# dlavado/scene-net

Hardware: AMD Instinct MI355X
Metric: voxel-tiles/sec (point cloud -> 64^3 occupancy -> 16-GENEO bank conv -> head) (higher is better)
Workload: dtype i8; 1 GPU; C2: 32 tiles/GPU x 100000 points (fp64 xyz, UTM-scale), 64^3 voxel grid, 16 GENEO kernels 9^3 (cy 6, cone 5, neg 5); conv on the int8 matrix cores: binary occupancy x 24-bit fixed-point weights (3 int8 digits), exact int32 accumulation, fp32 head; tiles_per_gpu=32, points_per_tile=100000, geneo_kernels=16, parallelism=tile-sharded x1, no collectives

## Files before the change

### include/scenenet_hip.h

```cpp
#ifndef SCENENET_HIP_H
#define SCENENET_HIP_H

#include <stddef.h>
#include <stdint.h>

#ifdef __cplusplus
extern "C" {
#endif

typedef void* sn_stream_t;

typedef enum {
    SN_OK = 0,
    SN_ERR_INVALID_ARG = -1,
    SN_ERR_UNSUPPORTED = -2,
    SN_ERR_LAUNCH = -3,
    SN_ERR_NO_DEVICE = -4,
    SN_ERR_DEVICE_STATUS = -5
} sn_status;

typedef enum { SN_F32 = 0, SN_F64 = 1, SN_U8 = 2, SN_OCC8 = 3, SN_BF16 = 4, SN_I32 = 5 } sn_dtype;

typedef enum {
    SN_GENEO_CY = 0, SN_GENEO_CONE = 1, SN_GENEO_NEG = 2,
    SN_GENEO_CY_V1 = 3, SN_GENEO_CONE_V1 = 4, SN_GENEO_NEG_V1 = 5
} sn_geneo_kind;

enum {
    SN_P_RADIUS = 0,
    SN_P_SIGMA = 1,
    SN_P_APEX = 2,
    SN_P_CONE_RADIUS = 3,
    SN_P_CONE_INC = 4,
    SN_P_NEG_FACTOR = 5,
    SN_NPARAM = 8
};

int sn_version(void);
int sn_prepare_device(void);
int sn_device_status(int* code, int* detail2);
int sn_device_status_clear(void);
int sn_conv_i8_path_counts(unsigned long long* counts3);
const char* sn_last_error(void);

int sn_device_count(void);

int sn_set_option(const char* name, int value);
int sn_get_option(const char* name);

int sn_geneo_bank(const float* params, const int32_t* kinds, int G, int kz, int kx, int ky,
                  float* bank, int32_t* status, sn_stream_t stream);

int sn_effective_lambdas(float* lambdas, const int32_t* order, int G, int last, float* out, sn_stream_t stream);
int sn_geneo_bank_lambdas(const float* params, const int32_t* kinds, int G, int kz, int kx, int ky, float* bank,
                          int32_t* status, float* lambdas, const int32_t* order, int last, float* lambdas_out,
                          sn_stream_t stream);
int sn_geneo_bank_prep(const float* params, const int32_t* kinds, int G, int kz, int kx, int ky, float* bank,
                       int32_t* status, float* lambdas, const int32_t* order, int last, float* lambdas_out,
                       void* prep, sn_stream_t stream);

int sn_conv_bank(const void* x, int x_dtype, const float* bank, const float* lambdas,
                 int B, int Z, int X, int Y, int G, int kz, int kx, int ky,
                 void* act, void* out, int out_dtype, sn_stream_t stream);

int sn_conv_bank_plan(int x_dtype, int B, int Z, int X, int Y, int G, int kz, int kx, int ky, int32_t* plan8);

#define SN_CONV_PREP_BYTES 16384
int sn_conv_bank_prep(const float* bank, int G, int kz, int kx, int ky, void* prep, sn_stream_t stream);
int sn_conv_bank_prepared(const void* x, int x_dtype, const float* bank, const float* lambdas, void* prep,
                          int B, int Z, int X, int Y, int G, int kz, int kx, int ky,
                          void* act, void* out, int out_dtype, sn_stream_t stream);
int sn_conv_bank_prepared_served(const void* x, int x_dtype, const float* bank, const float* lambdas, void* prep,
                                 int B, int Z, int X, int Y, int G, int kz, int kx, int ky,
                                 void* act, void* out, int out_dtype, sn_stream_t stream);
int sn_conv_prep_verdict_offset(void);
int sn_conv_i8_spin_timeouts(unsigned long long* count);
int sn_conv_i8z_round_counts(unsigned long long* counts2);
int sn_voxel_onepass_giveups(unsigned long long* count);

int sn_launch_timing_events(void* start_event, void* stop_event);

int sn_conv_fused(const void* x, int x_dtype, const float* bank, const float* lambdas, int B, int Z, int X, int Y,
                  int G, int kz, int kx, int ky, void* out, int out_dtype, sn_stream_t stream);
int sn_conv_fused_v(const void* x, int x_dtype, const float* bank, const float* lambdas, int B, int Z, int X, int Y, int G,
                    int kz, int kx, int ky, void* out, int out_dtype, int32_t* verdict, int assume_served,
                    sn_stream_t stream);
size_t sn_conv_fused_prep_bytes(int kz, int kx, int ky);
int sn_conv_fused_prep(const float* bank, const float* lambdas, int G, int kz, int kx, int ky, void* blob,
                       sn_stream_t stream);
int sn_conv_fused_prepared(const void* x, int x_dtype, const float* bank, const float* lambdas, const void* blob, int B,
                           int Z, int X, int Y, int G, int kz, int kx, int ky, void* out, int out_dtype, int assume_served,
                           sn_stream_t stream);


int sn_conv_fused_supported(int B, int Z, int X, int Y, int kz, int kx, int ky);

int sn_forward_auto(const void* x, int x_dtype, const float* bank, const float* lambdas, int B, int Z, int X, int Y,
                    int G, int kz, int kx, int ky, uint8_t* occ_ws, int32_t* not_binary, void* out, int out_dtype,
                    sn_stream_t stream);


#define SN_DESC_LEN(nx, ny, nz) (6 + (nx) + (ny) + (nz) + 3)

int sn_voxel_bbox(const double* pts, const int64_t* offsets, int B, double* bbox, sn_stream_t stream);

#define SN_BBOX_PARTS 32
int sn_voxel_prepare(const double* pts, const int64_t* offsets, int B, int nx, int ny, int nz, int regular,
                     double* partial_ws, double* bbox, double* desc, sn_stream_t stream);

int sn_voxel_desc(const double* bbox, int B, int nx, int ny, int nz, int regular,
                  double* desc, sn_stream_t stream);

int sn_voxel_desc_from_bounds(const double* bounds, int B, int nx, int ny, int nz,
                              double* desc, sn_stream_t stream);

int sn_voxel_desc_sized(const double* bbox, int B, const double* size_xyz_host, int nx, int ny, int nz,
                        double* desc, int32_t* dims, int32_t* status, sn_stream_t stream);

int sn_voxel_finalize_sized(const int32_t* counts, const int32_t* tower_counts, int B, int nx, int ny, int nz,
                            const double* desc, int32_t* colstats, double* density, double* gt, float* occ,
                            float* gt_occ, sn_stream_t stream);

int sn_voxel_scatter(const double* pts, const double* labels, const int64_t* offsets, int B,
                     const double* desc, int nx, int ny, int nz,
                     int32_t* counts, int32_t* tower_counts,
                     const double* keep_labels_host, int n_keep,
                     int32_t* dropped, sn_stream_t stream);

int sn_voxel_finalize(const int32_t* counts, const int32_t* tower_counts, int B, int nx, int ny, int nz,
                      int32_t* colstats, double* density, double* gt, float* occ, float* gt_occ,
                      sn_stream_t stream);

#define SN_OCC_PARTS 16
#define SN_OCC_WS_WORDS(B, V, planes) ((size_t)(B) * SN_OCC_PARTS * ((planes) * ((V) / 32) + 1))
int sn_voxel_occupancy(const double* pts, const double* labels, const int64_t* offsets, int B,
                       const double* desc, int nx, int ny, int nz,
                       const double* keep_labels_host, int n_keep,
                       uint32_t* bits_ws, void* occ, void* gt_occ, int out_dtype,
                       int32_t* flags, int32_t* dropped,
                       int32_t* counts_ws, int32_t* towers_ws, sn_stream_t stream);

int sn_voxel_occupancy_fused(const double* pts, const double* labels, const int64_t* offsets, int B, int nx, int ny,
                             int nz, int regular, const double* keep_labels_host, int n_keep, double* partial_ws,
                             double* bbox, double* desc, uint32_t* bits_ws, void* occ, void* gt_occ, int out_dtype,
                             int32_t* flags, int32_t* dropped, int32_t* counts_ws, int32_t* towers_ws,
                             sn_stream_t stream);

int sn_voxel_occupancy_fused_bank(const double* pts, const double* labels, const int64_t* offsets, int B, int nx, int ny,
                                  int nz, int regular, const double* keep_labels_host, int n_keep, double* partial_ws,
                                  double* bbox, double* desc, uint32_t* bits_ws, void* occ, void* gt_occ, int out_dtype,
                                  int32_t* flags, int32_t* dropped, int32_t* counts_ws, int32_t* towers_ws,
                                  const float* params, const int32_t* kinds, int G, int kz, int kx, int ky, float* bank,
                                  int32_t* status, float* lambdas, const int32_t* order, int last, float* lambdas_out,
                                  void* prep, sn_stream_t stream);

int sn_voxel_occupancy_sized(const double* pts, const double* labels, const int64_t* offsets, int B,
                             const double* size_xyz_host, int nx, int ny, int nz,
                             const double* keep_labels_host, int n_keep, double* partial_ws, double* bbox,
                             double* desc, int32_t* dims, int32_t* status, uint32_t* bits_ws, void* occ,
                             void* gt_occ, int out_dtype, int32_t* flags, int32_t* dropped,
                             int32_t* counts_ws, int32_t* towers_ws, sn_stream_t stream);
int sn_voxel_occupancy_sized_bank(const double* pts, const double* labels, const int64_t* offsets, int B,
                                  const double* size_xyz_host, int nx, int ny, int nz, const double* keep_labels_host,
                                  int n_keep, double* partial_ws, double* bbox, double* desc, int32_t* dims, int32_t* status,
                                  uint32_t* bits_ws, void* occ, void* gt_occ, int out_dtype, int32_t* flags,
                                  int32_t* dropped, int32_t* counts_ws, int32_t* towers_ws, const float* params,
                                  const int32_t* kinds, int G, int kz, int kx, int ky, float* bank, int32_t* bank_status,
                                  float* lambdas, const int32_t* order, int last, float* lambdas_out, void* prep,
                                  sn_stream_t stream);


int sn_gather_points(const void* grid, int dtype, int channels, const double* pts, const int64_t* offsets, int B,
                     const double* desc, int nx, int ny, int nz, double fill, void* out, sn_stream_t stream);

int sn_grid_to_points(const void* grid, int dtype, int n0, int n1, int n2, const double* origin_host,
                      const double* voxel_size_host, double* out, sn_stream_t stream);


int sn_conv_corr(const void* x, int x_dtype, const float* gout, const float* out, int B, int Z, int X, int Y,
                 int kz, int kx, int ky, float* partial_ws, float* C, sn_stream_t stream);
int sn_conv_corr_blocks(int B, int Z, int X, int Y);
int sn_conv_corr_t(const void* x, int x_dtype, const void* gout, const void* out, int g_dtype, int B, int Z, int X, int Y,
                   int kz, int kx, int ky, float* partial_ws, float* C, sn_stream_t stream);

size_t sn_conv_corr_ws_bytes(int x_dtype, int B, int Z, int X, int Y, int kz, int kx, int ky);
int sn_conv_corr_ws(const void* x, int x_dtype, const void* gout, const void* out, int g_dtype, int B, int Z, int X,
                    int Y, int kz, int kx, int ky, void* ws, size_t ws_bytes, float* C, sn_stream_t stream);

int sn_conv_corr_plan(int x_dtype, int g_dtype, int B, int Z, int X, int Y, int kz, int kx, int ky, int32_t* plan8);

int sn_geneo_bank_bwd(const float* params, const int32_t* kinds, int G, int kz, int kx, int ky,
                      const float* dW, float* dparams, sn_stream_t stream);

int sn_geneo_backward(const float* params, const int32_t* kinds, int G, int kz, int kx, int ky, const float* bank,
                      const float* lambdas, const float* corr, int last, float* dparams, float* dlambdas,
                      sn_stream_t stream);

#define SN_LOSS_MAX_BINS 16
#define SN_LOSS_NSTAT(H) (3 * (H) + 5)
#define SN_LOSS_PARTS(n_per) ((n_per) <= 16384 ? 1 : ((n_per) >= 16384 * 256 ? 256 : (int)(((n_per) + 16383) / 16384)))
#define SN_LOSS_WS_DOUBLES(B, n_per, H) ((int64_t)(B) * SN_LOSS_PARTS(n_per) * SN_LOSS_NSTAT(H))
#define SN_LOSS_NCOEF(B) (2 * SN_LOSS_MAX_BINS + 3 * (B))
typedef enum { SN_LOSS_WMSE = 1, SN_LOSS_FOCAL_TVERSKY = 2, SN_LOSS_DICE = 4, SN_LOSS_WBCE = 8 } sn_loss_term;

int sn_loss_forward(const void* pred, int pred_dtype, const void* gt, int gt_dtype, int B, int64_t n_per,
                    const float* ranges, const float* bin_w, int H, int terms, double mse_weight,
                    double tversky_alpha, double tversky_beta, double focal_gamma, double tversky_smooth,
                    double dice_smooth, double* parts_ws, double* stats, double* loss, double* coef,
                    sn_stream_t stream);

int sn_param_penalty(const float* P, const int8_t* mask, int N, float weight, int with_sum, float* value, float* grad,
                     sn_stream_t stream);

int sn_loss_backward(const void* pred, int pred_dtype, const void* gt, int gt_dtype, int B, int64_t n_per,
                     const float* ranges, int H, const double* coef, const double* upstream, void* grad_pred,
                     sn_stream_t stream);
int sn_loss_forward_m(const void* pred, int pred_dtype, const void* gt, int gt_dtype, int B, int64_t n_per,
                      const float* ranges, const float* bin_w, int H, int terms, double mse_weight, double tversky_alpha,
                      double tversky_beta, double focal_gamma, double tversky_smooth, double dice_smooth, double* parts_ws,
                      double* stats, double* loss, float* loss_f32, double* coef, sn_stream_t stream);
int sn_loss_backward_u(const void* pred, int pred_dtype, const void* gt, int gt_dtype, int B, int64_t n_per,
                       const float* ranges, int H, const double* coef, const void* upstream, int up_dtype, void* grad_pred,
                       sn_stream_t stream);
int sn_criterion_forward(const void* pred, int pred_dtype, const void* gt, int gt_dtype, int B, int64_t n_per,
                         const float* ranges, const float* bin_w, int H, int terms, double mse_weight, double tversky_alpha,
                         double tversky_beta, double focal_gamma, double tversky_smooth, double dice_smooth,
                         double* parts_ws, double* stats, double* loss, float* loss_f32, double* coef, const float* P,
                         const int8_t* mask, int N, float weight, int with_sum, float* pen_value, float* pen_grad,
                         float* total_f32, sn_stream_t stream);
int sn_criterion_backward(const void* pred, int pred_dtype, const void* gt, int gt_dtype, int B, int64_t n_per,
                          const float* ranges, int H, const double* coef, const void* upstream, int up_dtype,
                          void* grad_pred, const float* pen_grad, int N, float* pen_out, sn_stream_t stream);


#define SN_METRIC_NCOUNT 6
#define SN_METRIC_NVALUE 5
#define SN_METRIC_MAX_PARTS 1024
#define SN_METRIC_WS_BYTES (SN_METRIC_MAX_PARTS * SN_METRIC_NCOUNT * 8)

int sn_binary_stats(const void* pred, int pred_dtype, const void* target, int target_dtype, int64_t n, double tau,
                    double beta, void* parts_ws, uint64_t* state, uint64_t* batch, float* values, sn_stream_t stream);

#define SN_CURVE_MAX_THRESHOLDS 255
#define SN_CURVE_RECORD(T) (2 * ((T) + 1) + 2)
size_t sn_binary_curve_ws_bytes(int64_t n, int S, int T);
int sn_binary_curve(const void* pred, int pred_dtype, const void* target, int target_dtype, int64_t n, int S,
                    const double* thresholds_host, int T, void* parts_ws, size_t ws_bytes, uint64_t* state,
                    uint64_t* batch, sn_stream_t stream);



int sn_tiles_unpack(const void* rows, int row_dtype, int cols, int64_t total, const int64_t* offsets, int B,
                    double* pts, double* labels, int32_t* bad, sn_stream_t stream);


#define SN_TOWER_NSTAT 12
#define SN_TOWER_LAUNCHES 6

int sn_towers_stencil(double eps, const double* voxel_size_host, int32_t* rows_host, int cap, int64_t* n_offsets);

size_t sn_towers_ws_bytes(int B, int n0, int n1, int n2);

int sn_tower_proposals(const void* grid, int dtype, int B, int n0, int n1, int n2, double tau, double eps,
                       const double* voxel_size_host, int min_points, int max_towers, void* ws, size_t ws_bytes,
                       int32_t* labels, int32_t* n_towers, int64_t* stats, sn_stream_t stream);

int sn_tower_proposals_launches(const void* grid, int dtype, int B, int n0, int n1, int n2, double tau, double eps,
                                const double* voxel_size_host, int min_points, int max_towers, void* ws, size_t ws_bytes,
                                int32_t* labels, int32_t* n_towers, int64_t* stats, int first, int last,
                                sn_stream_t stream);


#define SN_CROP_DISC 0
#define SN_CROP_BOX 1

size_t sn_crops_ws_bytes(int64_t n, int K);
int sn_crops_chunk_points(void);

int sn_crop_count(const double* pts, int64_t n, const double* regions, const int32_t* kinds, int K, void* ws,
                  size_t ws_bytes, int64_t* offsets, sn_stream_t stream);

int sn_crop_scatter(const double* pts, const double* labels, int64_t n, const double* regions, const int32_t* kinds, int K,
                    const void* ws, size_t ws_bytes, const int64_t* offsets, int64_t capacity, double* out_pts,
                    double* out_labels, int64_t* out_src, sn_stream_t stream);


#define SN_CENSUS_MAX_WATCH 16

size_t sn_crop_census_ws_bytes(int64_t n, int K, int C);
int sn_census_chunk_points(void);

int sn_crop_census(const double* pts, const double* labels, int64_t n, const double* regions, const int32_t* kinds, int K,
                   const double* watch, int C, void* ws, size_t ws_bytes, int64_t* counts, double* label_range,
                   sn_stream_t stream);


#define SN_DBSCAN_NSTAT 3
#define SN_DBSCAN_LAUNCHES 8

int sn_points_select_chunk_points(void);
int sn_dbscan_chunk_points(void);

size_t sn_points_select_ws_bytes(int64_t n);

int sn_points_select(const double* pts, const double* labels, int64_t n, const double* keep, int n_keep, int64_t capacity,
                     void* ws, size_t ws_bytes, int64_t* sel, int64_t* n_sel, double* bbox, sn_stream_t stream);

int sn_dbscan_cell_grid(const double* bounds_host, double eps, int64_t max_cells, int32_t* dims_out, double* side_out);

size_t sn_dbscan_ws_bytes(int64_t capacity, int64_t cells);

int sn_dbscan_points(const double* pts, int64_t n, const int64_t* sel, const int64_t* n_sel, int64_t capacity,
                     const double* bounds_host, double eps, int min_points, int64_t max_cells, int max_clusters, void* ws,
                     size_t ws_bytes, int32_t* cluster, int32_t* n_clusters, int64_t* stats, int32_t* status,
                     sn_stream_t stream);

int sn_dbscan_points_launches(const double* pts, int64_t n, const int64_t* sel, const int64_t* n_sel, int64_t capacity,
                              const double* bounds_host, double eps, int min_points, int64_t max_cells, int max_clusters,
                              void* ws, size_t ws_bytes, int32_t* cluster, int32_t* n_clusters, int64_t* stats,
                              int32_t* status, int first, int last, sn_stream_t stream);


#define SN_TSCORE_MAX_ROWS 1024
#define SN_TSCORE_NTOTAL 8

int sn_tower_centroids(const int64_t* stats, const int32_t* n_towers, int B, int max_towers, int height_axis,
                       const double* voxel_size_host, const double* center_host, int apply_filter, double threshold,
                       double tower_height, double rim_sq, double min_euc, uint8_t* keep, double* planar, double* agg,
                       int32_t* n_agg, int32_t* status, sn_stream_t stream);

int sn_tower_match(const double* agg, const int32_t* n_agg, const int32_t* status_pred, int max_rows_pred,
                   const int64_t* gt_stats, const int32_t* gt_n_towers, int max_towers_gt, int B, int height_axis,
                   const double* voxel_size_host, double hit_dist, int32_t* match, double* dist, double* gt_planar,
                   int64_t* totals, double* dist_total, sn_stream_t stream);



int sn_las_chunk_records(void);

int sn_las_decode(const void* records, int64_t n, int point_format, int record_length, const double scale[3],
                  const double offset[3], double* pts, double* classes, int64_t* hist, sn_stream_t stream);



int sn_kitti_chunk_points(void);

int sn_kitti_decode(const void* scans, const void* label_words, int64_t total, const int64_t* offsets, int B,
                    const int32_t* lut, int n_lut, double* pts, double* labels, float* remission, int32_t* instance,
                    int64_t* hist, int n_hist, int32_t* bad, int32_t* unmapped, sn_stream_t stream);



int sn_las_encode_chunk_records(void);

int sn_las_encode(const double* pts, const double* classes, const uint16_t* intensity, const double* gps_time,
                  const uint16_t* rgb, int64_t n, int point_format, int record_length, const double scale[3],
                  const double offset[3], void* records, int32_t* box, int64_t* hist, int64_t* bad, sn_stream_t stream);


#define SN_CLOUD_DENSITY 0
#define SN_CLOUD_RANGES 1

int sn_voxel_cloud_chunk_cells(void);
size_t sn_voxel_cloud_ws_bytes(int B, int64_t V);

int sn_voxel_cloud_count(const void* grid, int dtype, int B, int n0, int n1, int n2, int mode, int r, const double* desc,
                         void* ws, size_t ws_bytes, int64_t* offsets, int64_t* bad, sn_stream_t stream);

int sn_voxel_cloud_scatter(const void* grid, int dtype, int B, int n0, int n1, int n2, int mode, int r,
                           const double* table_host, const double* desc, const void* ws, size_t ws_bytes,
                           const int64_t* offsets, int64_t capacity, double* rows, double* xyz, uint16_t* rgb16,
                           sn_stream_t stream);


#define SN_THIN_GROUP_NONE 0
#define SN_THIN_GROUP_Z 1
#define SN_THIN_GROUP_VOXEL 2

// ... 44 lines not shown
```

### scene-net_amd/_hip.py

```python
from __future__ import annotations

import contextlib
import ctypes
import functools
import os
from ctypes import c_char_p, c_int, c_void_p
from typing import NamedTuple, Optional, Sequence, Tuple

import torch

_HERE = os.path.dirname(os.path.abspath(__file__))
LIB_PATH = os.environ.get("SN_HIP_LIB") or os.path.join(_HERE, "lib", "libscenenet_hip.so")

SN_F32, SN_F64, SN_U8, SN_OCC8, SN_BF16, SN_I32 = 0, 1, 2, 3, 4, 5
SN_GENEO_CY, SN_GENEO_CONE, SN_GENEO_NEG = 0, 1, 2
SN_GENEO_CY_V1, SN_GENEO_CONE_V1, SN_GENEO_NEG_V1 = 3, 4, 5
SN_P_RADIUS, SN_P_SIGMA, SN_P_APEX, SN_P_CONE_RADIUS, SN_P_CONE_INC, SN_P_NEG_FACTOR = 0, 1, 2, 3, 4, 5
SN_NPARAM = 8

_P, _I = c_void_p, c_int
SYMBOLS = {
    "sn_version": (c_int, []),
    "sn_prepare_device": (c_int, []),
    "sn_device_status": (c_int, [_P, _P]),
    "sn_device_status_clear": (c_int, []),
    "sn_last_error": (c_char_p, []),
    "sn_device_count": (c_int, []),
    "sn_conv_i8_path_counts": (c_int, [_P]),
    "sn_set_option": (c_int, [c_char_p, _I]),
    "sn_get_option": (c_int, [c_char_p]),
    "sn_geneo_bank": (c_int, [_P, _P, _I, _I, _I, _I, _P, _P, _P]),
    "sn_effective_lambdas": (c_int, [_P, _P, _I, _I, _P, _P]),
    "sn_conv_bank": (c_int, [_P, _I, _P, _P, _I, _I, _I, _I, _I, _I, _I, _I, _P, _P, _I, _P]),
    "sn_conv_bank_plan": (c_int, [_I, _I, _I, _I, _I, _I, _I, _I, _I, _P]),
    "sn_geneo_bank_prep": (c_int, [_P, _P, _I, _I, _I, _I, _P, _P, _P, _P, _I, _P, _P, _P]),
    "sn_conv_bank_prep": (c_int, [_P, _I, _I, _I, _I, _P, _P]),
    "sn_conv_bank_prepared": (c_int, [_P, _I, _P, _P, _P, _I, _I, _I, _I, _I, _I, _I, _I, _P, _P, _I, _P]),
    "sn_conv_bank_prepared_served": (c_int, [_P, _I, _P, _P, _P, _I, _I, _I, _I, _I, _I, _I, _I, _P, _P, _I, _P]),
    "sn_conv_prep_verdict_offset": (c_int, []),
    "sn_conv_i8_spin_timeouts": (c_int, [_P]),
    "sn_conv_i8z_round_counts": (c_int, [_P]),
    "sn_voxel_onepass_giveups": (c_int, [_P]),
    "sn_launch_timing_events": (c_int, [_P, _P]),
    "sn_conv_fused": (c_int, [_P, _I, _P, _P, _I, _I, _I, _I, _I, _I, _I, _I, _P, _I, _P]),
    "sn_conv_fused_supported": (c_int, [_I, _I, _I, _I, _I, _I, _I]),
    "sn_forward_auto": (c_int, [_P, _I, _P, _P, _I, _I, _I, _I, _I, _I, _I, _I, _P, _P, _P, _I, _P]),
    "sn_voxel_bbox": (c_int, [_P, _P, _I, _P, _P]),
    "sn_voxel_desc": (c_int, [_P, _I, _I, _I, _I, _I, _P, _P]),
    "sn_voxel_desc_from_bounds": (c_int, [_P, _I, _I, _I, _I, _P, _P]),
    "sn_voxel_desc_sized": (c_int, [_P, _I, _P, _I, _I, _I, _P, _P, _P, _P]),
    "sn_voxel_finalize_sized": (c_int, [_P, _P, _I, _I, _I, _I, _P, _P, _P, _P, _P, _P, _P]),
    "sn_voxel_scatter": (c_int, [_P, _P, _P, _I, _P, _I, _I, _I, _P, _P, _P, _I, _P, _P]),
    "sn_voxel_finalize": (c_int, [_P, _P, _I, _I, _I, _I, _P, _P, _P, _P, _P, _P]),
    "sn_voxel_occupancy": (c_int, [_P, _P, _P, _I, _P, _I, _I, _I, _P, _I, _P, _P, _P, _I, _P, _P, _P, _P, _P]),
    "sn_voxel_occupancy_fused": (c_int, [_P, _P, _P, _I, _I, _I, _I, _I, _P, _I, _P, _P, _P, _P, _P, _P, _I, _P, _P, _P, _P,
                                         _P]),
    "sn_voxel_occupancy_fused_bank": (c_int, [_P, _P, _P, _I, _I, _I, _I, _I, _P, _I, _P, _P, _P, _P, _P, _P, _I, _P, _P, _P,
                                              _P, _P, _P, _I, _I, _I, _I, _P, _P, _P, _P, _I, _P, _P, _P]),
    "sn_voxel_occupancy_sized": (c_int, [_P, _P, _P, _I, _P, _I, _I, _I, _P, _I, _P, _P, _P, _P, _P, _P, _P, _P, _I, _P, _P,
                                         _P, _P, _P]),
    "sn_voxel_occupancy_sized_bank": (c_int, [_P, _P, _P, _I, _P, _I, _I, _I, _P, _I, _P, _P, _P, _P, _P, _P, _P, _P, _I, _P,
                                              _P, _P, _P, _P, _P, _I, _I, _I, _I, _P, _P, _P, _P, _I, _P, _P, _P]),
    "sn_voxel_prepare": (c_int, [_P, _P, _I, _I, _I, _I, _I, _P, _P, _P, _P]),
    "sn_gather_points": (c_int, [_P, _I, _I, _P, _P, _I, _P, _I, _I, _I, ctypes.c_double, _P, _P]),
    "sn_grid_to_points": (c_int, [_P, _I, _I, _I, _I, _P, _P, _P, _P]),
    "sn_conv_corr": (c_int, [_P, _I, _P, _P, _I, _I, _I, _I, _I, _I, _I, _P, _P, _P]),
    "sn_conv_corr_t": (c_int, [_P, _I, _P, _P, _I, _I, _I, _I, _I, _I, _I, _I, _P, _P, _P]),
    "sn_conv_corr_blocks": (c_int, [_I, _I, _I, _I]),
    "sn_conv_corr_ws_bytes": (ctypes.c_size_t, [_I, _I, _I, _I, _I, _I, _I, _I]),
    "sn_conv_corr_ws": (c_int, [_P, _I, _P, _P, _I, _I, _I, _I, _I, _I, _I, _I, _P, ctypes.c_size_t, _P, _P]),
    "sn_conv_corr_plan": (c_int, [_I, _I, _I, _I, _I, _I, _I, _I, _I, _P]),
    "sn_geneo_bank_lambdas": (c_int, [_P, _P, _I, _I, _I, _I, _P, _P, _P, _P, _I, _P, _P]),
    "sn_geneo_bank_bwd": (c_int, [_P, _P, _I, _I, _I, _I, _P, _P, _P]),
    "sn_geneo_backward": (c_int, [_P, _P, _I, _I, _I, _I, _P, _P, _P, _I, _P, _P, _P]),
    "sn_loss_forward": (c_int, [_P, _I, _P, _I, _I, ctypes.c_int64, _P, _P, _I, _I] + [ctypes.c_double] * 6
                        + [_P, _P, _P, _P, _P]),
    "sn_param_penalty": (c_int, [_P, _P, _I, ctypes.c_float, _I, _P, _P, _P]),
    "sn_loss_backward": (c_int, [_P, _I, _P, _I, _I, ctypes.c_int64, _P, _I, _P, _P, _P, _P]),
    "sn_conv_fused_prep_bytes": (ctypes.c_size_t, [_I, _I, _I]),
    "sn_conv_fused_prep": (c_int, [_P, _P, _I, _I, _I, _I, _P, _P]),
    "sn_conv_fused_prepared": (c_int, [_P, _I, _P, _P, _P, _I, _I, _I, _I, _I, _I, _I, _I, _P, _I, _I, _P]),
    "sn_conv_fused_v": (c_int, [_P, _I, _P, _P, _I, _I, _I, _I, _I, _I, _I, _I, _P, _I, _P, _I, _P]),
    "sn_loss_forward_m": (c_int, [_P, _I, _P, _I, _I, ctypes.c_int64, _P, _P, _I, _I] + [ctypes.c_double] * 6
                          + [_P, _P, _P, _P, _P, _P]),
    "sn_loss_backward_u": (c_int, [_P, _I, _P, _I, _I, ctypes.c_int64, _P, _I, _P, _P, _I, _P, _P]),
    "sn_criterion_forward": (c_int, [_P, _I, _P, _I, _I, ctypes.c_int64, _P, _P, _I, _I] + [ctypes.c_double] * 6
                             + [_P, _P, _P, _P, _P, _P, _P, _I, ctypes.c_float, _I, _P, _P, _P, _P]),
    "sn_criterion_backward": (c_int, [_P, _I, _P, _I, _I, ctypes.c_int64, _P, _I, _P, _P, _I, _P, _P, _I, _P, _P]),
    "sn_binary_stats": (c_int, [_P, _I, _P, _I, ctypes.c_int64, ctypes.c_double, ctypes.c_double, _P, _P, _P, _P, _P]),
    "sn_binary_curve_ws_bytes": (ctypes.c_size_t, [ctypes.c_int64, _I, _I]),
    "sn_binary_curve": (c_int, [_P, _I, _P, _I, ctypes.c_int64, _I, _P, _I, _P, ctypes.c_size_t, _P, _P, _P]),
    "sn_tiles_unpack": (c_int, [_P, _I, _I, ctypes.c_int64, _P, _I, _P, _P, _P, _P]),
    "sn_towers_stencil": (c_int, [ctypes.c_double, _P, _P, _I, _P]),
    "sn_towers_ws_bytes": (ctypes.c_size_t, [_I, _I, _I, _I]),
    "sn_tower_proposals": (c_int, [_P, _I, _I, _I, _I, _I, ctypes.c_double, ctypes.c_double, _P, _I, _I, _P,
                                   ctypes.c_size_t, _P, _P, _P, _P]),
    "sn_tower_proposals_launches": (c_int, [_P, _I, _I, _I, _I, _I, ctypes.c_double, ctypes.c_double, _P, _I, _I, _P,
                                            ctypes.c_size_t, _P, _P, _P, _I, _I, _P]),
    "sn_crops_ws_bytes": (ctypes.c_size_t, [ctypes.c_int64, _I]),
    "sn_crops_chunk_points": (c_int, []),
    "sn_crop_count": (c_int, [_P, ctypes.c_int64, _P, _P, _I, _P, ctypes.c_size_t, _P, _P]),
    "sn_crop_scatter": (c_int, [_P, _P, ctypes.c_int64, _P, _P, _I, _P, ctypes.c_size_t, _P, ctypes.c_int64, _P, _P, _P,
                                _P]),
    "sn_crop_census_ws_bytes": (ctypes.c_size_t, [ctypes.c_int64, _I, _I]),
    "sn_census_chunk_points": (c_int, []),
    "sn_crop_census": (c_int, [_P, _P, ctypes.c_int64, _P, _P, _I, _P, _I, _P, ctypes.c_size_t, _P, _P, _P]),
    "sn_points_select_chunk_points": (c_int, []),
    "sn_dbscan_chunk_points": (c_int, []),
    "sn_points_select_ws_bytes": (ctypes.c_size_t, [ctypes.c_int64]),
    "sn_points_select": (c_int, [_P, _P, ctypes.c_int64, _P, _I, ctypes.c_int64, _P, ctypes.c_size_t, _P, _P, _P, _P]),
    "sn_dbscan_cell_grid": (c_int, [_P, ctypes.c_double, ctypes.c_int64, _P, _P]),
    "sn_dbscan_ws_bytes": (ctypes.c_size_t, [ctypes.c_int64, ctypes.c_int64]),
    "sn_dbscan_points": (c_int, [_P, ctypes.c_int64, _P, _P, ctypes.c_int64, _P, ctypes.c_double, _I, ctypes.c_int64, _I, _P,
                                 ctypes.c_size_t, _P, _P, _P, _P, _P]),
    "sn_dbscan_points_launches": (c_int, [_P, ctypes.c_int64, _P, _P, ctypes.c_int64, _P, ctypes.c_double, _I, ctypes.c_int64,
                                          _I, _P, ctypes.c_size_t, _P, _P, _P, _P, _I, _I, _P]),
    "sn_tower_centroids": (c_int, [_P, _P, _I, _I, _I, _P, _P, _I, ctypes.c_double, ctypes.c_double, ctypes.c_double,
                                   ctypes.c_double, _P, _P, _P, _P, _P, _P]),
    "sn_las_chunk_records": (c_int, []),
    "sn_las_decode": (c_int, [_P, ctypes.c_int64, _I, _I, _P, _P, _P, _P, _P, _P]),
    "sn_tower_match": (c_int, [_P, _P, _P, _I, _P, _P, _I, _I, _I, _P, ctypes.c_double, _P, _P, _P, _P, _P, _P]),
    "sn_kitti_chunk_points": (c_int, []),
    "sn_kitti_decode": (c_int, [_P, _P, ctypes.c_int64, _P, _I, _P, _I, _P, _P, _P, _P, _P, _I, _P, _P, _P]),
    "sn_las_encode_chunk_records": (c_int, []),
    "sn_las_encode": (c_int, [_P, _P, _P, _P, _P, ctypes.c_int64, _I, _I, _P, _P, _P, _P, _P, _P, _P]),
    "sn_voxel_cloud_chunk_cells": (c_int, []),
    "sn_voxel_cloud_ws_bytes": (ctypes.c_size_t, [_I, ctypes.c_int64]),
    "sn_voxel_cloud_count": (c_int, [_P, _I, _I, _I, _I, _I, _I, _I, _P, _P, ctypes.c_size_t, _P, _P, _P]),
    "sn_voxel_cloud_scatter": (c_int, [_P, _I, _I, _I, _I, _I, _I, _I, _P, _P, _P, ctypes.c_size_t, _P, ctypes.c_int64, _P, _P,
                                       _P, _P]),
    "sn_thin_ws_bytes": (ctypes.c_size_t, [ctypes.c_int64, _I]),
    "sn_thin_chunk_points": (c_int, []),
    "sn_thin_count": (c_int, [_P, _P, ctypes.c_int64, _I, _I, _P, _I, _I, _I, _P, _P, _P, _P, _P, ctypes.c_size_t, _P, _P, _P,
                              _P]),
    "sn_thin_scatter": (c_int, [_P, _P, _P, ctypes.c_int64, _I, _I, _P, _I, _I, _I, _P, _P, _P, _P, _P, ctypes.c_size_t,
                                ctypes.c_int64, _P, _P, _P, _P, _P]),
    "sn_voxel_classes_chunk_points": (c_int, []),
    "sn_class_chunk_points": (c_int, []),
    "sn_voxel_classes": (c_int, [_P, _P, _P, ctypes.c_int64, _I, _P, _I, _I, _I, _I, _P, _P, _P, _P]),
    "sn_class_census": (c_int, [_P, _P, ctypes.c_int64, _I, _P, _P, _P]),
    "sn_class_paint": (c_int, [_P, _P, ctypes.c_int64, _I, _P, _P, _I, _P, _P, _P, _I, _P, _P, _P]),
    "sn_scan_merge": (c_int, [_P, _I, _I, _I, _I, _I, _I, _P, _P, ctypes.c_int64, _P, _P, _P, _I, _I, ctypes.c_double, _P, _P,
                              _P]),
}
SN_CONV_PREP_BYTES = 16384
SN_LOSS_WMSE, SN_LOSS_FOCAL_TVERSKY, SN_LOSS_DICE, SN_LOSS_WBCE = 1, 2, 4, 8
SN_LOSS_MAX_BINS = 16
SN_OCC_PARTS = 16
SN_BBOX_PARTS = 32
SN_METRIC_NCOUNT, SN_METRIC_NVALUE, SN_METRIC_MAX_PARTS = 6, 5, 1024
SN_METRIC_WS_BYTES = SN_METRIC_MAX_PARTS * SN_METRIC_NCOUNT * 8
SN_CURVE_MAX_THRESHOLDS = 255
SN_TOWER_NSTAT, SN_TOWER_LAUNCHES, SN_TOWER_MAX_RADIUS = 12, 6, 10
SN_TSCORE_MAX_ROWS, SN_TSCORE_NTOTAL = 1024, 8
SN_CROP_DISC, SN_CROP_BOX = 0, 1
SN_CENSUS_MAX_WATCH = 16
SN_DBSCAN_NSTAT, SN_DBSCAN_LAUNCHES = 3, 8
SN_KITTI_MAX_LUT, SN_KITTI_MAX_HIST = 65536, 1024
SN_CLOUD_DENSITY, SN_CLOUD_RANGES, SN_CLOUD_MAX_R = 0, 1, 32
SN_THIN_GROUP_NONE, SN_THIN_GROUP_Z, SN_THIN_GROUP_VOXEL = 0, 1, 2
SN_CLASS_WORDS, SN_VOXEL_CLASSES_NO_SKIP = 2048, 1
SN_MERGE_MAX, SN_MERGE_MEAN, SN_MERGE_INTERIOR = 0, 1, 2
OCC_MAX_WORDS = 16 * 1024


class HipLibraryError(RuntimeError):
    pass


_lib = None


def load() -> ctypes.CDLL:
    global _lib
    if _lib is not None:
        return _lib
    if not os.path.exists(LIB_PATH):
        raise HipLibraryError(
            f"{LIB_PATH} not found: the HIP extension is not built (run `make` or __graft_entry__.build()). "
            "There is no CPU fallback for this path.")
    lib = ctypes.CDLL(LIB_PATH)
    for name, (res, args) in SYMBOLS.items():
        fn = getattr(lib, name)
        fn.restype = res
        fn.argtypes = args
    _lib = lib
    return lib


def _check(rc: int, what: str) -> None:
    if rc != 0:
        msg = load().sn_last_error()
        raise HipLibraryError(f"{what} failed ({rc}): {msg.decode() if msg else ''}")


def device_status() -> Tuple[int, int, int]:
    code = ctypes.c_int(0)
    detail = (ctypes.c_int * 2)(0, 0)
    _check_plain(load().sn_device_status(ctypes.byref(code), detail), "sn_device_status")
    return int(code.value), int(detail[0]), int(detail[1])


def device_status_clear() -> None:
    _check_plain(load().sn_device_status_clear(), "sn_device_status_clear")


def _check_plain(rc: int, what: str) -> None:
    if rc != 0:
        msg = load().sn_last_error()
        raise HipLibraryError(f"{what} failed ({rc}): {msg.decode() if msg else ''}")


def set_option(name: str, value: int) -> None:
    _check(load().sn_set_option(name.encode(), int(value)), "sn_set_option")


def get_option(name: str) -> int:
    return int(load().sn_get_option(name.encode()))


@contextlib.contextmanager
def options(**values: int):
    found = []
    for name in values:
        old = get_option(name)
        if old == -1:
            raise HipLibraryError(f"sn_get_option: unknown option '{name}'")
        found.append((name, old))
    try:
        for name, value in values.items():
            set_option(name, value)
        yield
    finally:
        for name, old in reversed(found):
            set_option(name, old)


def conv_i8_path_counts() -> Tuple[int, int, int]:
    buf = (ctypes.c_ulonglong * 3)()
    _check(load().sn_conv_i8_path_counts(ctypes.cast(buf, ctypes.c_void_p)), "sn_conv_i8_path_counts")
    return int(buf[0]), int(buf[1]), int(buf[2])


def conv_i8_spin_timeouts() -> int:
    buf = (ctypes.c_ulonglong * 1)()
    _check(load().sn_conv_i8_spin_timeouts(ctypes.cast(buf, ctypes.c_void_p)), "sn_conv_i8_spin_timeouts")
    return int(buf[0])


def conv_i8z_round_counts() -> Tuple[int, int]:
    buf = (ctypes.c_ulonglong * 2)()
    _check(load().sn_conv_i8z_round_counts(ctypes.cast(buf, ctypes.c_void_p)), "sn_conv_i8z_round_counts")
    return int(buf[0]), int(buf[1])


def voxel_onepass_giveups() -> int:
    buf = (ctypes.c_ulonglong * 1)()
    _check(load().sn_voxel_onepass_giveups(ctypes.cast(buf, ctypes.c_void_p)), "sn_voxel_onepass_giveups")
    return int(buf[0])


def launch_timing_events(start: "torch.cuda.Event", stop: "torch.cuda.Event") -> None:
    a, b = int(start.cuda_event), int(stop.cuda_event)
    if not a or not b:
        raise HipLibraryError("launch_timing_events: record each event once first (torch creates the handle lazily)")
    _check_plain(load().sn_launch_timing_events(ctypes.c_void_p(a), ctypes.c_void_p(b)), "sn_launch_timing_events")


def _ptr(t: Optional[torch.Tensor], dtype: Optional[torch.dtype] = None, name: str = "tensor") -> Optional[int]:
    if t is None:
        return None
    if not t.is_cuda:
        raise HipLibraryError(f"{name} must live on a HIP device (got {t.device}); there is no CPU path")
    if not t.is_contiguous():
        raise HipLibraryError(f"{name} must be contiguous")
    if dtype is not None and t.dtype != dtype:
        raise HipLibraryError(f"{name} must be {dtype} (got {t.dtype})")
    return t.data_ptr()


_raw_stream = getattr(torch._C, "_cuda_getCurrentRawStream", None)


def _stream() -> int:
    if _raw_stream is not None:
        return _raw_stream(torch.cuda.current_device())
    return torch.cuda.current_stream().cuda_stream


def _common_device(tensors) -> Optional[torch.device]:
    dev = None
    for t in tensors:
        if t is None or not getattr(t, "is_cuda", False):
            continue
        if dev is None:
            dev = t.device
        elif t.device != dev:
            raise HipLibraryError(f"tensor arguments live on different devices ({dev} and {t.device}); "
                                  "a call of the C ABI runs on one device and one stream")
    return dev


_get_device = getattr(torch._C, "_cuda_getDevice", None)


def _on_tensor_device(fn):
    @functools.wraps(fn)
    def wrapper(*args, **kwargs):
        idx = -1
        for a in args:
            if isinstance(a, torch.Tensor):
                d = a.get_device()
                if d >= 0:
                    if idx < 0:
                        idx = d
                    elif d != idx:
                        _common_device([t for t in args if isinstance(t, torch.Tensor)])
        if kwargs:
            for a in kwargs.values():
                if isinstance(a, torch.Tensor):
                    d = a.get_device()
                    if d >= 0:
                        if idx < 0:
                            idx = d
                        elif d != idx:
                            _common_device([t for t in list(args) + list(kwargs.values()) if isinstance(t, torch.Tensor)])
        if idx < 0 or idx == (_get_device() if _get_device is not None else torch.cuda.current_device()):
            return fn(*args, **kwargs)
        with torch.cuda.device(idx):
            return fn(*args, **kwargs)
    return wrapper


_DT = {torch.float32: SN_F32, torch.float64: SN_F64, torch.uint8: SN_U8, torch.bool: SN_OCC8, torch.bfloat16: SN_BF16}
_DT_OUT = {torch.float32: SN_F32, torch.float64: SN_F64, torch.uint8: SN_U8, torch.bool: SN_U8,
           torch.bfloat16: SN_BF16}


@_on_tensor_device
def geneo_bank(params: torch.Tensor, kinds: torch.Tensor, kernel_size: Sequence[int],
               status: Optional[torch.Tensor] = None, out: Optional[torch.Tensor] = None) -> torch.Tensor:
    G = params.shape[0]
    kz, kx, ky = (int(k) for k in kernel_size)
    if out is None:
        out = torch.empty((G, kz, kx, ky), dtype=torch.float32, device=params.device)
    rc = load().sn_geneo_bank(_ptr(params, torch.float32, "params"), _ptr(kinds, torch.int32, "kinds"), G, kz, kx, ky,
                              _ptr(out, torch.float32, "bank"), _ptr(status, torch.int32, "status"), _stream())
    _check(rc, "sn_geneo_bank")
    return out


@_on_tensor_device
def geneo_bank_lambdas(params: torch.Tensor, kinds: torch.Tensor, kernel_size: Sequence[int], lambdas: torch.Tensor,
                       order: torch.Tensor, last: int):
    G = params.shape[0]
    kz, kx, ky = (int(k) for k in kernel_size)
    bank = torch.empty((G, kz, kx, ky), dtype=torch.float32, device=params.device)
    lam = torch.empty((G,), dtype=torch.float32, device=params.device)
    rc = load().sn_geneo_bank_lambdas(_ptr(params, torch.float32, "params"), _ptr(kinds, torch.int32, "kinds"), G, kz,
                                      kx, ky, _ptr(bank), None, _ptr(lambdas, torch.float32, "lambdas"),
                                      _ptr(order, torch.int32, "order"), int(last), _ptr(lam), _stream())
    _check(rc, "sn_geneo_bank_lambdas")
    return bank, lam


@_on_tensor_device
def geneo_bank_prep(params: torch.Tensor, kinds: torch.Tensor, lambdas: Optional[torch.Tensor] = None,
                    order: Optional[torch.Tensor] = None, last: int = 0, bank: Optional[torch.Tensor] = None,
                    lam_out: Optional[torch.Tensor] = None, prep: Optional[torch.Tensor] = None):
    G = params.shape[0]
    if bank is None:
        bank = torch.empty((G, 9, 9, 9), dtype=torch.float32, device=params.device)
    nbytes = SN_CONV_PREP_BYTES * ((G + 15) // 16)
    if prep is None:
        prep = torch.empty(nbytes, dtype=torch.uint8, device=params.device)
    if lambdas is not None and lam_out is None:
        lam_out = torch.empty(G, dtype=torch.float32, device=params.device)
    rc = load().sn_geneo_bank_prep(_ptr(params, torch.float32, "params"), _ptr(kinds, torch.int32, "kinds"), G, 9, 9, 9,
                                   _ptr(bank, torch.float32, "bank"), None, _ptr(lambdas, torch.float32, "lambdas"),
                                   _ptr(order, torch.int32, "order"), int(last), _ptr(lam_out, torch.float32, "lam_out"),
                                   _ptr(prep, torch.uint8, "prep"), _stream())
    _check(rc, "sn_geneo_bank_prep")
    return bank, (lam_out if lambdas is not None else None), prep


def prep_verdicts(prep: torch.Tensor) -> torch.Tensor:
    off = int(load().sn_conv_prep_verdict_offset())
    return prep.view(-1, SN_CONV_PREP_BYTES)[:, off:off + 4].view(torch.int32).reshape(-1)


class PreparedVerdict:

    def __init__(self):
        self._key = None
        self._state = 0
        self._host = None
        self._event = None

    def __reduce__(self):
        return (PreparedVerdict, ())

    def served(self, key) -> bool:
        if torch.cuda.is_current_stream_capturing():
            return False
        if key != self._key:
            self._key, self._state = key, 0
            return False
        if self._state == 1 and self._event.query():
            if int(self._host.min()) < 0:
                self._state = 0
            else:
                self._state = 2 if int(self._host.max()) == 0 else 3
        return self._state == 2

    def note(self, prep: torch.Tensor, key) -> None:
        self.note_words(prep_verdicts(prep), key)

    def note_words(self, words: torch.Tensor, key) -> None:
        if key != self._key or self._state != 0 or torch.cuda.is_current_stream_capturing():
            return
        if self._host is None or self._host.numel() != words.numel():
            self._host = torch.empty(words.numel(), dtype=torch.int32, pin_memory=True)
        self._host.copy_(words, non_blocking=True)
        self._event = torch.cuda.Event()
        self._event.record()
        self._state = 1


@_on_tensor_device
def conv_bank_prep(bank: torch.Tensor, prep: Optional[torch.Tensor] = None) -> torch.Tensor:
    G, kz, kx, ky = bank.shape
    nbytes = SN_CONV_PREP_BYTES * ((G + 15) // 16)
    if prep is None:
        prep = torch.empty(nbytes, dtype=torch.uint8, device=bank.device)
    elif prep.dtype != torch.uint8 or prep.numel() < nbytes:
        raise HipLibraryError(f"prep must be uint8 with at least {nbytes} bytes")
    rc = load().sn_conv_bank_prep(_ptr(bank, torch.float32, "bank"), G, kz, kx, ky, _ptr(prep, torch.uint8, "prep"),
                                  _stream())
    _check(rc, "sn_conv_bank_prep")
    return prep


@_on_tensor_device
def conv_bank(x: torch.Tensor, bank: torch.Tensor, lambdas: Optional[torch.Tensor], want_act: bool = False,
              want_out: bool = True, out_dtype: Optional[torch.dtype] = None, prep: Optional[torch.Tensor] = None,
              assume_served: bool = False):
    if x.dim() != 5 or x.shape[1] != 1:
        raise HipLibraryError(f"x must be [B,1,Z,X,Y] (got {tuple(x.shape)})")
    if x.dtype not in _DT or x.dtype == torch.bfloat16:
        raise HipLibraryError(f"x dtype {x.dtype} unsupported (f32, f64, u8, bool)")
    B, _, Z, X, Y = x.shape
    G, kz, kx, ky = bank.shape
    if out_dtype is None:
        out_dtype = x.dtype if x.dtype in (torch.float32, torch.float64) else torch.float32
    act = torch.empty((B, G, Z, X, Y), dtype=out_dtype, device=x.device) if want_act else None
    out = torch.empty((B, 1, Z, X, Y), dtype=out_dtype, device=x.device) if want_out else None
    if prep is not None:
        if prep.dtype != torch.uint8 or prep.numel() < SN_CONV_PREP_BYTES * ((G + 15) // 16):
            raise HipLibraryError("prep: not a blob of conv_bank_prep for this bank")
        fn = load().sn_conv_bank_prepared_served if assume_served else load().sn_conv_bank_prepared
        rc = fn(_ptr(x, None, "x"), _DT[x.dtype], _ptr(bank, torch.float32, "bank"),
                _ptr(lambdas, torch.float32, "lambdas"), _ptr(prep, torch.uint8, "prep"),
                B, Z, X, Y, G, kz, kx, ky, _ptr(act, None, "act"), _ptr(out, None, "out"),
                _DT_OUT[out_dtype], _stream())
        _check(rc, "sn_conv_bank_prepared")
        return act, out
    rc = load().sn_conv_bank(_ptr(x, None, "x"), _DT[x.dtype], _ptr(bank, torch.float32, "bank"),
                             _ptr(lambdas, torch.float32, "lambdas"), B, Z, X, Y, G, kz, kx, ky,
                             _ptr(act, None, "act"), _ptr(out, None, "out"), _DT_OUT[out_dtype], _stream())
    _check(rc, "sn_conv_bank")
    return act, out


class ConvPlan(NamedTuple):
    kernel: str
    tz: int
    tx: int
    ntiles: int
    double_buffered: bool
    staged: bool
    row_stride: int
    cus: int

    @property
    def rung(self) -> Tuple[int, int]:
        return (self.tz, self.tx)


CONV_PLAN_KERNELS = ("fp32", "four_copy", "stride4", "folded")


def conv_bank_plan(x, bank_shape: Sequence[int]) -> ConvPlan:
    dtype, shape = (x.dtype, tuple(x.shape)) if isinstance(x, torch.Tensor) else (x[0], tuple(x[1]))
    if len(shape) != 5 or shape[1] != 1:
        raise HipLibraryError(f"x must be [B,1,Z,X,Y] (got {shape})")
    if dtype not in _DT or dtype == torch.bfloat16:
        raise HipLibraryError(f"x dtype {dtype} unsupported (f32, f64, u8, bool)")
    B, _, Z, X, Y = (int(v) for v in shape)
    G, kz, kx, ky = (int(v) for v in bank_shape)
    p = (ctypes.c_int32 * 8)()
    _check(load().sn_conv_bank_plan(_DT[dtype], B, Z, X, Y, G, kz, kx, ky, ctypes.cast(p, c_void_p)), "sn_conv_bank_plan")
    return ConvPlan(CONV_PLAN_KERNELS[p[0]], int(p[1]), int(p[2]), int(p[3]), bool(p[4] & 1), bool(p[4] & 2), int(p[5]),
                    int(p[6]))


def conv_fused_supported(x: torch.Tensor, kernel_size: Sequence[int]) -> bool:
    if x.dtype != torch.bool or x.dim() != 5:
        return False
    kz, kx, ky = (int(k) for k in kernel_size)
    B, _, Z, X, Y = x.shape
    return bool(load().sn_conv_fused_supported(int(B), int(Z), int(X), int(Y), kz, kx, ky))


@_on_tensor_device
def conv_fused(x: torch.Tensor, bank: torch.Tensor, lambdas: torch.Tensor,
               out_dtype: torch.dtype = torch.float32, verdict: Optional[torch.Tensor] = None,
               assume_served: bool = False, prep: Optional[torch.Tensor] = None) -> torch.Tensor:
    B, _, Z, X, Y = x.shape
    G, kz, kx, ky = bank.shape
    out = torch.empty((B, 1, Z, X, Y), dtype=out_dtype, device=x.device)
    if prep is not None:
        rc = load().sn_conv_fused_prepared(_ptr(x, None, "x"), _DT[x.dtype], _ptr(bank, torch.float32, "bank"),
                                           _ptr(lambdas, torch.float32, "lambdas"), _ptr(prep, torch.uint8, "prep"), B, Z,
                                           X, Y, G, kz, kx, ky, _ptr(out), _DT_OUT[out_dtype], int(bool(assume_served)),
                                           _stream())
        _check(rc, "sn_conv_fused_prepared")
        return out
    if verdict is None:
        rc = load().sn_conv_fused(_ptr(x, None, "x"), _DT[x.dtype], _ptr(bank, torch.float32, "bank"),
                                  _ptr(lambdas, torch.float32, "lambdas"), B, Z, X, Y, G, kz, kx, ky, _ptr(out),
                                  _DT_OUT[out_dtype], _stream())
    else:
        rc = load().sn_conv_fused_v(_ptr(x, None, "x"), _DT[x.dtype], _ptr(bank, torch.float32, "bank"),
                                    _ptr(lambdas, torch.float32, "lambdas"), B, Z, X, Y, G, kz, kx, ky, _ptr(out),
                                    _DT_OUT[out_dtype], _ptr(verdict, torch.int32, "verdict"), int(bool(assume_served)),
                                    _stream())
    _check(rc, "sn_conv_fused")
    return out


def conv_fused_prep_bytes(kernel_size: Sequence[int]) -> int:
    kz, kx, ky = (int(k) for k in kernel_size)
    return int(load().sn_conv_fused_prep_bytes(kz, kx, ky))


@_on_tensor_device
def conv_fused_prep(bank: torch.Tensor, lambdas: torch.Tensor, blob: Optional[torch.Tensor] = None) -> torch.Tensor:
    G, kz, kx, ky = bank.shape
    nbytes = conv_fused_prep_bytes((kz, kx, ky))
    if nbytes == 0:
        raise HipLibraryError(f"sn_conv_fused_prep: kernel {kz}x{kx}x{ky} is outside the combined kernel")
    if blob is None:
        blob = torch.empty(nbytes, dtype=torch.uint8, device=bank.device)
    elif blob.dtype != torch.uint8 or blob.numel() < nbytes:
        raise HipLibraryError(f"blob must be uint8 with at least {nbytes} bytes")
    _check(load().sn_conv_fused_prep(_ptr(bank, torch.float32, "bank"), _ptr(lambdas, torch.float32, "lambdas"), G, kz, kx,
                                     ky, _ptr(blob, torch.uint8, "blob"), _stream()), "sn_conv_fused_prep")
    return blob


def conv_fused_prep_verdict(blob: torch.Tensor, kernel_size: Sequence[int]) -> torch.Tensor:
    n = conv_fused_prep_bytes(kernel_size)
    return blob[n - 12:n - 8].view(torch.int32)


@_on_tensor_device
def forward_auto(x: torch.Tensor, bank: torch.Tensor, lambdas: torch.Tensor, out_dtype: Optional[torch.dtype] = None):
    B, _, Z, X, Y = x.shape
    G, kz, kx, ky = bank.shape
    out_dtype = x.dtype if out_dtype is None else out_dtype
    if x.data_ptr() % 16:
        x = x.clone()
    out = torch.empty((B, 1, Z, X, Y), dtype=out_dtype, device=x.device)
    occ = torch.empty((x.numel(),), dtype=torch.uint8, device=x.device)
    flag = torch.empty((1,), dtype=torch.int32, device=x.device)
    rc = load().sn_forward_auto(_ptr(x, None, "x"), _DT[x.dtype], _ptr(bank, torch.float32, "bank"),
                                _ptr(lambdas, torch.float32, "lambdas"), B, Z, X, Y, G, kz, kx, ky, _ptr(occ), _ptr(flag),
                                _ptr(out), _DT_OUT[out_dtype], _stream())
    _check(rc, "sn_forward_auto")
    return out, flag


def desc_len(nx: int, ny: int, nz: int) -> int:
    return 6 + nx + ny + nz + 3


@_on_tensor_device
def voxel_bbox(pts: torch.Tensor, offsets: torch.Tensor) -> torch.Tensor:
    B = offsets.numel() - 1
    bbox = torch.empty((B, 6), dtype=torch.float64, device=pts.device)
    rc = load().sn_voxel_bbox(_ptr(pts, torch.float64, "pts"), _ptr(offsets, torch.int64, "offsets"), B,
                              _ptr(bbox), _stream())
    _check(rc, "sn_voxel_bbox")
    return bbox


@_on_tensor_device
def voxel_prepare(pts: torch.Tensor, offsets: torch.Tensor, n_xyz: Sequence[int], regular: bool = True,
                  want_bbox: bool = False):
    B = offsets.numel() - 1
    nx, ny, nz = (int(v) for v in n_xyz)
    dev = pts.device
    partial = torch.empty((B, SN_BBOX_PARTS, 6), dtype=torch.float64, device=dev)
    desc = torch.empty((B, desc_len(nx, ny, nz)), dtype=torch.float64, device=dev)
    bbox = torch.empty((B, 6), dtype=torch.float64, device=dev) if want_bbox else None
    rc = load().sn_voxel_prepare(_ptr(pts, torch.float64, "pts"), _ptr(offsets, torch.int64, "offsets"), B, nx, ny, nz,
                                 int(regular), _ptr(partial), _ptr(bbox), _ptr(desc), _stream())
    _check(rc, "sn_voxel_prepare")
    return desc, bbox


@_on_tensor_device
def voxel_desc(bbox: torch.Tensor, n_xyz: Sequence[int], regular: bool = True, from_bounds: bool = False):
    B = bbox.shape[0]
    nx, ny, nz = (int(v) for v in n_xyz)
    desc = torch.empty((B, desc_len(nx, ny, nz)), dtype=torch.float64, device=bbox.device)
    if from_bounds:
        rc = load().sn_voxel_desc_from_bounds(_ptr(bbox, torch.float64, "bounds"), B, nx, ny, nz, _ptr(desc),
                                              _stream())
    else:
        rc = load().sn_voxel_desc(_ptr(bbox, torch.float64, "bbox"), B, nx, ny, nz, int(regular), _ptr(desc),
                                  _stream())
    _check(rc, "sn_voxel_desc")
    return desc


@_on_tensor_device
def voxel_desc_sized(bbox: torch.Tensor, voxel_dims: Sequence[float], max_n_xyz: Sequence[int]):
    B = bbox.shape[0]
    nx, ny, nz = (int(v) for v in max_n_xyz)
    dev = bbox.device
    desc = torch.empty((B, desc_len(nx, ny, nz)), dtype=torch.float64, device=dev)
    dims = torch.empty((B, 3), dtype=torch.int32, device=dev)
    status = torch.empty((B,), dtype=torch.int32, device=dev)
    if len(voxel_dims) != 3:
        raise HipLibraryError("voxel_dims must have 3 entries (size_x, size_y, size_z)")
    sz = (ctypes.c_double * 3)(*[float(v) for v in voxel_dims])
    rc = load().sn_voxel_desc_sized(_ptr(bbox, torch.float64, "bbox"), B, ctypes.cast(sz, c_void_p), nx, ny, nz,
                                    _ptr(desc), _ptr(dims), _ptr(status), _stream())
    _check(rc, "sn_voxel_desc_sized")
    return desc, dims, status


@_on_tensor_device
def voxel_finalize_sized(counts, towers, desc, want_density=False, want_gt=False, want_occ=True, want_gt_occ=False):
    B, nz, nx, ny = counts.shape
    dev = counts.device
    shape = (B, 1, nz, nx, ny)
    colstats = torch.empty((B, 2, ny), dtype=torch.int32, device=dev) if (want_density or want_occ) else None
    density = torch.empty(shape, dtype=torch.float64, device=dev) if want_density else None
    gt = torch.empty(shape, dtype=torch.float64, device=dev) if want_gt else None
    occ = torch.empty(shape, dtype=torch.float32, device=dev) if want_occ else None
    gt_occ = torch.empty(shape, dtype=torch.float32, device=dev) if want_gt_occ else None
    rc = load().sn_voxel_finalize_sized(_ptr(counts, torch.int32, "counts"), _ptr(towers, torch.int32, "towers"), B, nx,
                                        ny, nz, _ptr(desc, torch.float64, "desc"), _ptr(colstats), _ptr(density),
                                        _ptr(gt), _ptr(occ), _ptr(gt_occ), _stream())
    _check(rc, "sn_voxel_finalize_sized")
    return density, gt, occ, gt_occ


@_on_tensor_device
def voxel_scatter(pts, labels, offsets, desc, n_xyz, keep_labels: Sequence[float] = (), want_towers: bool = False,
                  counts=None, towers=None, dropped=None):
    B = offsets.numel() - 1
    nx, ny, nz = (int(v) for v in n_xyz)
    dev = pts.device
    if counts is None:
        counts = torch.empty((B, nz, nx, ny), dtype=torch.int32, device=dev)
    if want_towers and towers is None:
        towers = torch.empty((B, nz, nx, ny), dtype=torch.int32, device=dev)
    if dropped is None:
        dropped = torch.empty((B,), dtype=torch.int32, device=dev)
    keep = (ctypes.c_double * max(1, len(keep_labels)))(*[float(k) for k in keep_labels])
    rc = load().sn_voxel_scatter(_ptr(pts, torch.float64, "pts"), _ptr(labels, torch.float64, "labels"),
                                 _ptr(offsets, torch.int64, "offsets"), B, _ptr(desc, torch.float64, "desc"),
                                 nx, ny, nz, _ptr(counts, torch.int32, "counts"),
                                 _ptr(towers, torch.int32, "towers") if want_towers else None,
                                 ctypes.cast(keep, c_void_p), len(keep_labels), _ptr(dropped), _stream())
    _check(rc, "sn_voxel_scatter")
    return counts, (towers if want_towers else None), dropped


@_on_tensor_device
def voxel_finalize(counts, towers, want_density=False, want_gt=False, want_occ=True, want_gt_occ=False):
    B, nz, nx, ny = counts.shape
    dev = counts.device
    shape = (B, 1, nz, nx, ny)
    colstats = torch.empty((B, 2, ny), dtype=torch.int32, device=dev) if (want_density or want_occ) else None
    density = torch.empty(shape, dtype=torch.float64, device=dev) if want_density else None
    gt = torch.empty(shape, dtype=torch.float64, device=dev) if want_gt else None
    occ = torch.empty(shape, dtype=torch.float32, device=dev) if want_occ else None
    gt_occ = torch.empty(shape, dtype=torch.float32, device=dev) if want_gt_occ else None
    rc = load().sn_voxel_finalize(_ptr(counts, torch.int32, "counts"), _ptr(towers, torch.int32, "towers"), B, nx, ny,
                                  nz, _ptr(colstats), _ptr(density), _ptr(gt), _ptr(occ), _ptr(gt_occ), _stream())
    _check(rc, "sn_voxel_finalize")
    return density, gt, occ, gt_occ


def occupancy_supported(n_xyz: Sequence[int], planes: int) -> bool:
    nx, ny, nz = (int(v) for v in n_xyz)
    V = nx * ny * nz
    if V % 32:
        return False
    sl = 1
    while sl <= SN_OCC_PARTS:
        if nz % sl == 0 and (V // 32) % sl == 0 and ((nz // sl) * nx * ny) % 32 == 0 \
                and (V // 32 // sl) * planes <= OCC_MAX_WORDS:
            return True
        sl *= 2
    return False


@_on_tensor_device
def voxel_occupancy(pts, labels, offsets, desc, n_xyz, keep_labels: Sequence[float] = (), want_gt_occ: bool = False,
                    out_dtype: torch.dtype = torch.uint8, exact_fallback: bool = True):
    B = offsets.numel() - 1
    nx, ny, nz = (int(v) for v in n_xyz)
    V = nx * ny * nz
    dev = pts.device
    planes = 2 if want_gt_occ else 1
    bits = torch.empty((B * SN_OCC_PARTS * (planes * (V // 32) + 1),), dtype=torch.int32, device=dev)
    occ = torch.empty((B, 1, nz, nx, ny), dtype=out_dtype, device=dev)
    gt_occ = torch.empty((B, 1, nz, nx, ny), dtype=out_dtype, device=dev) if want_gt_occ else None
    flags = torch.empty((B,), dtype=torch.int32, device=dev)
    dropped = torch.empty((B,), dtype=torch.int32, device=dev)
    counts = towers = None
    if exact_fallback:
        counts = torch.empty((B, V), dtype=torch.int32, device=dev)
        towers = torch.empty((B, V), dtype=torch.int32, device=dev) if want_gt_occ else None
    keep = (ctypes.c_double * max(1, len(keep_labels)))(*[float(k) for k in keep_labels])
    rc = load().sn_voxel_occupancy(_ptr(pts, torch.float64, "pts"),
                                   _ptr(labels, torch.float64, "labels") if want_gt_occ else None,
                                   _ptr(offsets, torch.int64, "offsets"), B, _ptr(desc, torch.float64, "desc"),
                                   nx, ny, nz, ctypes.cast(keep, c_void_p), len(keep_labels) if want_gt_occ else 0,
                                   _ptr(bits), _ptr(occ), _ptr(gt_occ), _DT_OUT[out_dtype], _ptr(flags), _ptr(dropped),
                                   _ptr(counts), _ptr(towers), _stream())
    _check(rc, "sn_voxel_occupancy")
    return occ, gt_occ, flags, dropped


@_on_tensor_device
def voxel_occupancy_fused(pts, labels, offsets, n_xyz, regular: bool = True, keep_labels: Sequence[float] = (),
                          want_gt_occ: bool = False, out_dtype: torch.dtype = torch.uint8, exact_fallback: bool = True,
                          want_bbox: bool = False, bank_rider=None):
    B = offsets.numel() - 1
    nx, ny, nz = (int(v) for v in n_xyz)
    V = nx * ny * nz
    dev = pts.device
    planes = 2 if want_gt_occ else 1
    partial = torch.empty((B, SN_BBOX_PARTS, 6), dtype=torch.float64, device=dev)
    desc = torch.empty((B, desc_len(nx, ny, nz)), dtype=torch.float64, device=dev)
    bbox = torch.empty((B, 6), dtype=torch.float64, device=dev) if want_bbox else None
    bits = torch.empty((B * SN_OCC_PARTS * (planes * (V // 32) + 1),), dtype=torch.int32, device=dev)
    occ = torch.empty((B, 1, nz, nx, ny), dtype=out_dtype, device=dev)
    gt_occ = torch.empty((B, 1, nz, nx, ny), dtype=out_dtype, device=dev) if want_gt_occ else None
    flags = torch.empty((B,), dtype=torch.int32, device=dev)
    dropped = torch.empty((B,), dtype=torch.int32, device=dev)
    counts = towers = None
    if exact_fallback:
        counts = torch.empty((B, V), dtype=torch.int32, device=dev)
        towers = torch.empty((B, V), dtype=torch.int32, device=dev) if want_gt_occ else None
    keep = (ctypes.c_double * max(1, len(keep_labels)))(*[float(k) for k in keep_labels])
    common = (_ptr(pts, torch.float64, "pts"), _ptr(labels, torch.float64, "labels") if want_gt_occ else None,
              _ptr(offsets, torch.int64, "offsets"), B, nx, ny, nz, int(regular), ctypes.cast(keep, c_void_p),
              len(keep_labels) if want_gt_occ else 0, _ptr(partial), _ptr(bbox), _ptr(desc), _ptr(bits), _ptr(occ),
              _ptr(gt_occ), _DT_OUT[out_dtype], _ptr(flags), _ptr(dropped), _ptr(counts), _ptr(towers))
    if bank_rider is None:
        rc = load().sn_voxel_occupancy_fused(*common, _stream())
# ... 1023 lines not shown
```

### scene-net_amd/csrc/cabi.hip

```cpp
#include "common.h"
#include <climits>
#include <cstdlib>
#include <cstring>

#include <atomic>
#include <mutex>
#include <unordered_map>

namespace sn {
char* error_buffer() {
    static thread_local char buf[512] = {0};
    return buf;
}
namespace {
struct Option {
    const char* name;
    const char* env;
    int on;
    int def, lo, hi;
    bool is_switch;
    std::atomic<int> value{env ? -1 : def};
};
Option g_options[] = {
    {"conv_skip_empty_tiles",  nullptr,                 0,  0,       0,  1,       true},
    {"conv_i8_tolerance_ppb",  nullptr,                 0,  90000,   0,  INT_MAX, false},
    {"conv_i8_fold",           "SN_CONV_I8_NOFOLD",     0,  1,       0,  1,       true},
    {"conv_i8_legacy",         "SN_CONV_I8_LEGACY",     1,  0,       0,  1,       true},
    {"conv_i8_no_stage",       "SN_CONV_I8_NO_STAGE",   1,  0,       0,  1,       true},
    {"conv_i8z_variant",       nullptr,                 0,  2,       0,  2,       false},
    {"conv_no_i8",             "SN_CONV_NO_I8",         1,  0,       0,  1,       true},
    {"conv_double_buffer",     "SN_CONV_DOUBLE_BUFFER", 1,  0,       0,  1,       true},
    {"conv_lin_no24",          "SN_CONV_LIN_NO24",      1,  0,       0,  1,       true},
    {"voxel_onepass",          nullptr,                 0,  1,       0,  1,       true},
    {"voxel_onepass_spin",     nullptr,                 0,  64,      0,  INT_MAX, false},
    {"corr_dense",             "SN_CORR_DENSE",         1,  0,       0,  1,       true},
    {"corr_sparse_tile_bytes", nullptr,                 0,  0,       0,  2048,    false},
    {"conv_i8z_inject_fault",  nullptr,                 0,  0,       0,  1,       true},
    {"conv_i8z_dense",         nullptr,                 0,  0,       0,  1,       true},
};
static_assert(sizeof(g_options) / sizeof(g_options[0]) == kOptCount, "one entry per sn::Opt");
}

int option(Opt which) {
    Option& o = g_options[which];
    int v = o.value.load(std::memory_order_relaxed);
    if (v < 0) {
        const char* e = getenv(o.env);
        int expected = -1;
        o.value.compare_exchange_strong(expected, (e && e[0] == '1') ? o.on : o.def, std::memory_order_relaxed);
        v = o.value.load(std::memory_order_relaxed);
    }
    return v;
}

static thread_local Gate g_gate{{nullptr, nullptr, nullptr}, {0, 0, 0}};
Gate current_gate() { return g_gate; }
GateScope::GateScope(const int32_t* ptr, int want) : slot_(-1) {
    for (int i = 0; i < kGateDepth; ++i)
        if (!g_gate.ptr[i]) { slot_ = i; break; }
    if (slot_ < 0) abort();
    g_gate.ptr[slot_] = ptr;
    g_gate.want[slot_] = want;
}
GateScope::~GateScope() {
    g_gate.ptr[slot_] = nullptr;
    g_gate.want[slot_] = 0;
}

namespace {
constexpr int kFlagRing = 1024, kFlagCapture = 4096, kFlagMaxDev = 16;
std::mutex g_flag_mu;
int32_t* g_flag_mem[kFlagMaxDev] = {nullptr};
unsigned g_flag_next[kFlagMaxDev] = {0}, g_flag_cap_next[kFlagMaxDev] = {0};
volatile int32_t* g_sticky_host[kFlagMaxDev] = {nullptr};
int32_t* g_sticky_dev[kFlagMaxDev] = {nullptr};
int32_t* flag_pool_locked(int dev) {
    if (!g_flag_mem[dev]) {
        if (hipMalloc((void**)&g_flag_mem[dev], (kFlagRing + kFlagCapture) * sizeof(int32_t)) != hipSuccess) {
            (void)hipGetLastError();
            g_flag_mem[dev] = nullptr;
            return nullptr;
        }
        (void)hipMemset(g_flag_mem[dev], 0, (kFlagRing + kFlagCapture) * sizeof(int32_t));
    }
    if (!g_sticky_host[dev]) {
        void* h = nullptr;
        void* d = nullptr;
        if (hipHostMalloc(&h, 16 * sizeof(int32_t), hipHostMallocMapped | hipHostMallocCoherent) == hipSuccess &&
            hipHostGetDevicePointer(&d, h, 0) == hipSuccess) {
            memset(h, 0, 16 * sizeof(int32_t));
            g_sticky_dev[dev] = static_cast<int32_t*>(d);
            g_sticky_host[dev] = static_cast<volatile int32_t*>(h);
        } else {
            (void)hipGetLastError();
        }
    }
    return g_flag_mem[dev];
}
}

namespace {
thread_local hipEvent_t g_timing_start = nullptr, g_timing_stop = nullptr;
}
void take_timing_events(hipEvent_t& start, hipEvent_t& stop) {
    start = g_timing_start;
    stop = g_timing_stop;
    g_timing_start = g_timing_stop = nullptr;
}

int32_t* sticky_device_ptr(hipStream_t stream) {
    int dev = 0;
    if (hipGetDevice(&dev) != hipSuccess || dev < 0 || dev >= kFlagMaxDev) return nullptr;
    if (g_sticky_dev[dev]) return g_sticky_dev[dev];
    hipStreamCaptureStatus st = hipStreamCaptureStatusNone;
    if (hipStreamIsCapturing(stream, &st) == hipSuccess && st == hipStreamCaptureStatusActive) return nullptr;
    (void)hipGetLastError();
    std::lock_guard<std::mutex> lock(g_flag_mu);
    (void)flag_pool_locked(dev);
    return g_sticky_dev[dev];
}

int sticky_check(const char* what) {
    for (int dev = 0; dev < kFlagMaxDev; ++dev) {
        volatile int32_t* w = g_sticky_host[dev];
        if (!w || w[0] == 0) continue;
        static const char* const kText[] = {"", "a dependency spin of the z-walk contraction gave up (its workgroup's outputs are NaN)",
                                            "a launch made with `assume served` was declined by the bank's guard (its outputs are NaN): "
                                            "a cached verdict did not belong to these parameters",
                                            "a hand-over spin of an int8 tile kernel gave up (that launch's output is not to be trusted)"};
        const int code = w[0];
        return fail(SN_ERR_DEVICE_STATUS, "%s: device %d has a latched status %d -- %s [workgroup %d, detail %d]; "
                    "sn_device_status_clear() re-arms the device", what, dev, code,
                    (code >= 1 && code <= 3) ? kText[code] : "unknown", (int)w[2], (int)w[3]);
    }
    return SN_OK;
}

int32_t* device_flag_slot(hipStream_t stream) {
    int dev = 0;
    if (hipGetDevice(&dev) != hipSuccess || dev < 0 || dev >= kFlagMaxDev) return nullptr;
    hipStreamCaptureStatus st = hipStreamCaptureStatusNone;
    const bool capturing = hipStreamIsCapturing(stream, &st) == hipSuccess && st == hipStreamCaptureStatusActive;
    if (!capturing) (void)hipGetLastError();
    std::lock_guard<std::mutex> lock(g_flag_mu);
    int32_t* mem = flag_pool_locked(dev);
    if (!mem) return nullptr;
    if (capturing && g_flag_cap_next[dev] < (unsigned)kFlagCapture) return mem + kFlagRing + g_flag_cap_next[dev]++;
    return mem + (g_flag_next[dev]++ % kFlagRing);
}

hipError_t ensure_dynamic_lds(const void* kernel, int bytes) {
    static std::mutex mu;
    static std::unordered_map<const void*, int> configured;
    std::lock_guard<std::mutex> lock(mu);
    int dev = 0;
    (void)hipGetDevice(&dev);
    const void* key = (const char*)kernel + dev;
    auto it = configured.find(key);
    if (it != configured.end() && it->second >= bytes) return hipSuccess;
    const hipError_t e = hipFuncSetAttribute(kernel, hipFuncAttributeMaxDynamicSharedMemorySize, bytes);
    if (e == hipSuccess) configured[key] = bytes;
    return e;
}
}

extern "C" int sn_set_option(const char* name, int value) {
    if (!name) return sn::fail(SN_ERR_INVALID_ARG, "sn_set_option: null name");
    for (auto& o : sn::g_options) {
        if (strcmp(name, o.name) != 0) continue;
        if (o.is_switch)
            value = value != 0;
        else if (value < o.lo || value > o.hi)
            return sn::fail(SN_ERR_INVALID_ARG, "sn_set_option: %s takes %d .. %d", name, o.lo, o.hi);
        o.value.store(value, std::memory_order_relaxed);
        return SN_OK;
    }
    return sn::fail(SN_ERR_INVALID_ARG, "sn_set_option: unknown option '%s'", name);
}

extern "C" int sn_get_option(const char* name) {
    for (int i = 0; name && i < sn::kOptCount; ++i)
        if (strcmp(name, sn::g_options[i].name) == 0) return sn::option(static_cast<sn::Opt>(i));
    return -1;
}

extern "C" int sn_prepare_device(void) {
    int dev = 0;
    if (hipGetDevice(&dev) != hipSuccess || dev < 0 || dev >= sn::kFlagMaxDev)
        return sn::fail(SN_ERR_NO_DEVICE, "sn_prepare_device: no current HIP device");
    std::lock_guard<std::mutex> lock(sn::g_flag_mu);
    return sn::flag_pool_locked(dev) ? SN_OK : sn::fail(SN_ERR_LAUNCH, "sn_prepare_device: cannot allocate the flag pool");
}

extern "C" int sn_device_status(int* code, int* detail2) {
    int dev = 0;
    if (hipGetDevice(&dev) != hipSuccess || dev < 0 || dev >= sn::kFlagMaxDev)
        return sn::fail(SN_ERR_NO_DEVICE, "sn_device_status: no current HIP device");
    volatile int32_t* w = sn::g_sticky_host[dev];
    if (code) *code = w ? (int)w[0] : 0;
    if (detail2) {
        detail2[0] = w ? (int)w[2] : 0;
        detail2[1] = w ? (int)w[3] : 0;
    }
    return SN_OK;
}

extern "C" int sn_launch_timing_events(void* start_event, void* stop_event) {
    sn::g_timing_start = static_cast<hipEvent_t>(start_event);
    sn::g_timing_stop = static_cast<hipEvent_t>(stop_event);
    return SN_OK;
}

extern "C" int sn_device_status_clear(void) {
    int dev = 0;
    if (hipGetDevice(&dev) != hipSuccess || dev < 0 || dev >= sn::kFlagMaxDev)
        return sn::fail(SN_ERR_NO_DEVICE, "sn_device_status_clear: no current HIP device");
    if (hipDeviceSynchronize() != hipSuccess) {
        const hipError_t e = hipGetLastError();
        return sn::fail(SN_ERR_LAUNCH, "sn_device_status_clear: %s", hipGetErrorString(e));
    }
    volatile int32_t* w = sn::g_sticky_host[dev];
    if (w) {
        w[0] = 0; w[2] = 0; w[3] = 0;
        w[1] = 0;
    }
    return SN_OK;
}

extern "C" int sn_version(void) { return 105; }

extern "C" const char* sn_last_error(void) { return sn::error_buffer(); }

extern "C" int sn_device_count(void) {
    int n = 0;
    if (hipGetDeviceCount(&n) != hipSuccess) {
        (void)hipGetLastError();
        return 0;
    }
    int ok = 0;
    for (int i = 0; i < n; ++i) {
        hipDeviceProp_t p;
        if (hipGetDeviceProperties(&p, i) == hipSuccess && strncmp(p.gcnArchName, "gfx950", 6) == 0) ++ok;
    }
    return ok;
}
```

### scene-net_amd/csrc/common.h

```cpp
#pragma once
#include <hip/hip_runtime.h>
#include <cstdarg>
#include <cstdio>
#include <cstdlib>
#include "scenenet_hip.h"

namespace sn {

char* error_buffer();

inline int fail(int code, const char* fmt, ...) {
    va_list ap;
    va_start(ap, fmt);
    vsnprintf(error_buffer(), 512, fmt, ap);
    va_end(ap);
    return code;
}

int sticky_check(const char* what);

inline int check_launch(const char* what) {
    hipError_t e = hipGetLastError();
    if (e != hipSuccess) return fail(SN_ERR_LAUNCH, "%s: %s", what, hipGetErrorString(e));
    return sticky_check(what);
}

inline hipStream_t as_stream(sn_stream_t s) { return reinterpret_cast<hipStream_t>(s); }

enum Opt {
    kOptConvSkipEmptyTiles,
    kOptConvI8TolerancePpb,
    kOptConvI8Fold,
    kOptConvI8Legacy,
    kOptConvI8NoStage,
    kOptConvI8zVariant,
    kOptConvNoI8,
    kOptConvDoubleBuffer,
    kOptConvLinNo24,
    kOptVoxelOnepass,
    kOptVoxelOnepassSpin,
    kOptCorrDense,
    kOptCorrSparseTileBytes,
    kOptConvI8zInjectFault,
    kOptConvI8zDense,
    kOptCount
};
int option(Opt which);
inline float conv_i8_tolerance() { return 1e-9f * (float)option(kOptConvI8TolerancePpb); }

hipError_t ensure_dynamic_lds(const void* kernel, int bytes);

constexpr int kGateDepth = 3;
struct Gate {
    const int32_t* ptr[kGateDepth];
    int want[kGateDepth];
    __device__ __forceinline__ bool pass() const {
#pragma unroll
        for (int i = 0; i < kGateDepth; ++i)
            if (ptr[i] && *ptr[i] != want[i]) return false;
        return true;
    }
};
Gate current_gate();
struct GateScope {
    GateScope(const int32_t* ptr, int want);
    ~GateScope();
  private:
    int slot_;
};

#ifdef SN_CONV_DEBUG
#define SN_DBG(shape, bit) (((shape).dbg & (bit)) != 0)
#else
#define SN_DBG(shape, bit) false
#endif
inline int debug_env_int(const char* name) {
#ifdef SN_CONV_DEBUG
    const char* v = getenv(name);
    return v ? atoi(v) : 0;
#else
    (void)name;
    return 0;
#endif
}

void take_timing_events(hipEvent_t& start, hipEvent_t& stop);
int32_t* sticky_device_ptr(hipStream_t stream);
int sticky_check(const char* what);
__device__ __forceinline__ void sticky_latch(int32_t* sticky, int code, int a, int b) {
    if (!sticky) return;
    a = __builtin_amdgcn_readfirstlane(a);
    b = __builtin_amdgcn_readfirstlane(b);
    asm volatile("" : "+s"(a), "+s"(b));
    if (__hip_atomic_exchange(&sticky[1], 1, __ATOMIC_RELAXED, __HIP_MEMORY_SCOPE_SYSTEM) == 0) {
        __hip_atomic_store(&sticky[2], a, __ATOMIC_RELAXED, __HIP_MEMORY_SCOPE_SYSTEM);
        __hip_atomic_store(&sticky[3], b, __ATOMIC_RELAXED, __HIP_MEMORY_SCOPE_SYSTEM);
        __hip_atomic_store(&sticky[0], code, __ATOMIC_RELEASE, __HIP_MEMORY_SCOPE_SYSTEM);
    }
}

__device__ __forceinline__ unsigned long long enc_f64(double d) {
    unsigned long long u = (unsigned long long)__double_as_longlong(d);
    return (u >> 63) ? ~u : (u | 0x8000000000000000ull);
}
__device__ __forceinline__ double dec_f64(unsigned long long u) {
    u = (u >> 63) ? (u & 0x7fffffffffffffffull) : ~u;
    return __longlong_as_double((long long)u);
}

__device__ __forceinline__ uint64_t widen_f32_bits(uint32_t u) {
    const uint64_t sign = (uint64_t)(u >> 31) << 63;
    const uint32_t e = (u >> 23) & 0xffu, m = u & 0x7fffffu;
    if (e == 0xffu) return sign | 0x7ff0000000000000ull | ((uint64_t)m << 29) | (m ? 0x0008000000000000ull : 0ull);
    if (e == 0) {
        if (m == 0) return sign;
        const int p = 31 - __clz((int)m);
        return sign | ((uint64_t)(p - 149 + 1023) << 52) | ((uint64_t)(m - (1u << p)) << (52 - p));
    }
    return sign | ((uint64_t)(e + (1023 - 127)) << 52) | ((uint64_t)m << 29);
}

int32_t* device_flag_slot(hipStream_t stream);

}
```

### scene-net_amd/csrc/conv_i8s.hip

```cpp
#include "common.h"
#include <hip/hip_ext.h>
#include <cstdlib>
#include <cstring>
#include <type_traits>
#include <vector>

namespace {

#include "conv_prep.h"
#include "conv_fp32.inc"

#include "conv_i8_common.inc"
#include "conv_i8s_kernel.inc"
#include "conv_i8f.inc"

size_t lds_bytes_fold(const Shape& s) {
    const size_t hdw = (size_t)s.ZP * s.XP * DW;
    const size_t ring = kNB * hdw * 4, alias = 2 * hdw * 4 + ((size_t)s.G * 729 + 1) * sizeof(float);
    return (size_t)kFoldSteps * 3 * 64 * 16 + 64 + 64 + 128 + 128 + 64 + sizeof(FoldPlan) +
           (ring > alias ? ring : alias) + 16;
}

void plan_fold(int XP, FoldPlan& p) {
    for (int qq = 0; qq < 4; ++qq) {
        auto put = [&](int slot, int dz, int dxp, bool pad) {
            p.h1[qq][slot] = (short)(dz * XP + dxp);
            p.h2[qq][slot] = (short)(dz * XP + 8 - dxp);
            p.tap[qq][slot] = pad ? (short)-1 : (short)(dz * 9 + dxp);
        };
        for (int slot = 0; slot < kFoldSlots; ++slot)
            if (!fold_slot_irregular(slot)) put(slot, 2 * qq + fold_slot_a(slot), fold_slot_dx(slot), false);
        static const int last_dx[4] = {0, 2, 1, 3};
        put(11, 8, last_dx[qq], false);
        static const int pad_dz[4] = {8, 6, 0, 2};
        put(8, pad_dz[qq], 4, qq != 0);
    }
}

size_t lds_bytes(const Shape& s) {
    const size_t hdw = (size_t)s.ZP * s.XP * DW;
    return (size_t)s.KS * 3 * 64 * 16 + (size_t)s.NP * 4 * 8 + (size_t)s.NT * 4 * 16 + 16 + 64 + 64 + 128 + 128 + 64 + sizeof(RowPlan) +
           (kNB * hdw * 4 > 2 * hdw * 4 + ((size_t)s.G * s.kz * s.kx * 9 + 1) * sizeof(float)
                ? kNB * hdw * 4 : 2 * hdw * 4 + ((size_t)s.G * s.kz * s.kx * 9 + 1) * sizeof(float)) + 16;
}

int num_cus() {
    static thread_local int cached = 0;
    if (cached) return cached;
    int dev = 0;
    hipDeviceProp_t p;
    if (hipGetDevice(&dev) != hipSuccess || hipGetDeviceProperties(&p, dev) != hipSuccess) {
        (void)hipGetLastError();
        return 256;
    }
    cached = p.multiProcessorCount > 0 ? p.multiProcessorCount : 256;
    return cached;
}

bool plan_rows(int kz, int kx, int XP, RowPlan& p, int& RQ) {
    const int R = kz * kx;
    RQ = (R + 3) / 4;
    if (RQ > kMaxRQ || RQ < 1) return false;
    static_assert((2 * DW) % 32 == 16, "plan_rows pairs halo rows 2 (mod 4) apart: 2 * DW must be 16 (mod 32) dwords");
    std::vector<int> cls[4];
    for (int dz = 0; dz < kz; ++dz)
        for (int dx = 0; dx < kx; ++dx) cls[(dz * XP + dx) & 3].push_back(dz * kx + dx);
    std::vector<std::pair<int, int>> units;
    std::vector<int> singles;
    for (int c = 0; c < 2; ++c) {
        const auto &a = cls[c], &b = cls[c + 2];
        const size_t m = a.size() < b.size() ? a.size() : b.size();
        for (size_t i = 0; i < m; ++i) units.emplace_back(a[i], b[i]);
        for (size_t i = m; i < a.size(); ++i) singles.push_back(a[i]);
        for (size_t i = m; i < b.size(); ++i) singles.push_back(b[i]);
    }
    for (size_t i = 0; i + 1 < singles.size(); i += 2) units.emplace_back(singles[i], singles[i + 1]);
    if (singles.size() & 1) units.emplace_back(singles.back(), -1);
    if ((int)units.size() > 2 * RQ) return false;
    auto halo_of = [&](int krow) { return (krow / kx) * XP + (krow % kx); };
    for (int qq = 0; qq < 4; ++qq)
        for (int i = 0; i < kMaxRQ; ++i) { p.halo[qq][i] = 0; p.tap[qq][i] = -1; }
    for (size_t u = 0; u < units.size(); ++u) {
        const int half = (int)(u & 1), pos = (int)(u >> 1);
        const int a = units[u].first, b = units[u].second;
        p.tap[2 * half][pos] = (short)a;
        p.halo[2 * half][pos] = (short)halo_of(a);
        p.tap[2 * half + 1][pos] = (short)b;
        p.halo[2 * half + 1][pos] = (short)(b >= 0 ? halo_of(b) : halo_of(a));
    }
    return true;
}

bool plan_stride4(Shape& s, int B, int Z, int X, int Y, int kz, int kx, int cus) {
    static const int cand[][2] = {{8, 8}, {4, 8}, {4, 4}, {2, 4}, {1, 4}, {1, 2}};
    bool found = false;
    for (const auto& c : cand) {
        s.TZ = c[0]; s.TX = c[1];
        s.nzt = (Z + s.TZ - 1) / s.TZ; s.nxt = (X + s.TX - 1) / s.TX;
        const long long nt = (long long)B * s.nzt * s.nxt * s.nyt;
        if (nt > 0x7fffffff) return false;
        s.ntiles = (int)nt;
        s.ZP = s.TZ + kz - 1;
        s.XP = (s.TX + kx - 1) | 1;
        if (!plan_rows(kz, kx, s.XP, s.plan, s.RQ)) return false;
        s.ODD = s.RQ & 1;
        s.NP = s.RQ / 2;
        s.NT = (s.RQ + 3) / 4;
        s.NTS = (s.NT + 2 * s.ODD + 3) / 4;
        s.KS = s.NP + s.NTS;
        if (s.NP != 10 || s.NT != 6 || s.ODD != 1) return false;
        if (s.ZP * s.XP > 32767) continue;
        if (lds_bytes(s) > (size_t)kMaxLds) continue;
        found = true;
        if (s.ntiles >= 4 * cus) break;
    }
    return found;
}

bool stride4_shape(int Y, int G, int kz, int kx, int ky) {
    if (ky != 9 || kz * kx != 81 || Y % 16 != 0 || G > 16) return false;
    return !sn::option(sn::kOptConvSkipEmptyTiles);
}

bool fold_fits(const Shape& s, size_t& ldsf) {
    ldsf = lds_bytes_fold(s) > lds_bytes(s) ? lds_bytes_fold(s) : lds_bytes(s);
    return s.kz == 9 && s.kx == 9 && sn::option(sn::kOptConvI8Fold) && ldsf <= (size_t)kMaxLds &&
           (s.XP == 17 || s.XP == 13 || s.XP == 11);
}

#include "conv_i8z.inc"

}

namespace sn {

int conv_bank_group(const void* x, int x_dtype, const float* bank, const float* lambdas, int B, int Z, int X, int Y,
                    int G, int Gtot, int g0, int head, int kz, int kx, int ky, void* act, void* out, int out_dtype,
                    sn_stream_t stream);
int conv_occ_i8s_plan(int B, int Z, int X, int Y, int G, int kz, int kx, int ky, int32_t* plan8);

int conv_occ_i8s(const uint8_t* x, const float* bank, const float* lambdas, int B, int Z, int X, int Y, int G, int Gtot,
                 int g0, int head, int kz, int kx, int ky, void* act, void* out, int out_dtype, hipStream_t stream) {
    if (!stride4_shape(Y, G, kz, kx, ky) || (reinterpret_cast<uintptr_t>(x) & 15) != 0) return 1;
    if (act && (reinterpret_cast<uintptr_t>(act) & 15)) return 1;
    if (out && (reinterpret_cast<uintptr_t>(out) & 15)) return 1;
    Shape s;
    memset(&s, 0, sizeof(s));
    s.B = B; s.Z = Z; s.X = X; s.Y = Y; s.G = G; s.kz = kz; s.kx = kx;
    s.Gtot = Gtot; s.g0 = g0; s.head = head;
    s.gate = sn::current_gate();
    s.sticky = sn::sticky_device_ptr(stream);
    s.nyt = (Y + TY - 1) / TY;
    s.dbg = sn::debug_env_int("SN_CONV_I8_DBG");
    s.stagger = sn::debug_env_int("SN_CONV_I8S_STAGGER");
    s.dynamic = !sn::debug_env_int("SN_CONV_I8S_STATIC");
    const int cus = num_cus();
    const bool found = plan_stride4(s, B, Z, X, Y, kz, kx, cus);
    if (!found) return 1;
    s.tol = sn::conv_i8_tolerance();
    const int grid = cus < s.ntiles ? cus : s.ntiles;
    int32_t* flag = sn::device_flag_slot(stream);
    size_t ldsf = 0;
    const bool fold = flag && s.dbg == 0 &&
                      fold_fits(s, ldsf);
    bool folded = false;
    if (fold) {
        Shape sf = s;
        plan_fold(sf.XP, sf.fplan);
        sf.route = flag;
#define SN_LAUNCH_I8F(OT, XPV)                                                                                   \
    do {                                                                                                         \
        auto kern = conv_occ_i8f_kernel<OT, XPV>;                                                                \
        if (sn::ensure_dynamic_lds((const void*)kern, kMaxLds) != hipSuccess)                                    \
            return check_launch("sn_conv_bank(i8f: hipFuncSetAttribute)");                                       \
        hipLaunchKernelGGL(kern, dim3(grid), dim3(kThreads), ldsf, stream, x, bank, lambdas, sf, (OT*)act,       \
                           (OT*)out);                                                                            \
    } while (0)
#define SN_LAUNCH_I8F_XP(XPV)                                                                                    \
    do {                                                                                                         \
        if (out_dtype == SN_F32) SN_LAUNCH_I8F(float, XPV);                                                      \
        else SN_LAUNCH_I8F(double, XPV);                                                                         \
    } while (0)
        if (sf.XP == 17) SN_LAUNCH_I8F_XP(17);
        else if (sf.XP == 13) SN_LAUNCH_I8F_XP(13);
        else SN_LAUNCH_I8F_XP(11);
#undef SN_LAUNCH_I8F_XP
#undef SN_LAUNCH_I8F
        if (int rc = check_launch("sn_conv_bank(i8f)")) return rc;
        folded = true;
    }
    s.route = folded ? flag : nullptr;
    if (!folded) {
        if (s.tol > 0.0f) {
            s.route = flag;
            if (!s.route) s.tol = 0.0f;
        }
        const size_t lds = lds_bytes(s);
#define SN_LAUNCH_I8S(OT)                                                                                        \
    do {                                                                                                         \
        auto kern = conv_occ_i8s_kernel<OT, 10, 6, 1>;                                                           \
        if (sn::ensure_dynamic_lds((const void*)kern, kMaxLds) != hipSuccess)                                    \
            return check_launch("sn_conv_bank(i8s: hipFuncSetAttribute)");                                       \
        hipLaunchKernelGGL(kern, dim3(grid), dim3(kThreads), lds, stream, x, bank, lambdas, s, (OT*)act,         \
                           (OT*)out);                                                                            \
    } while (0)
        if (out_dtype == SN_F32) SN_LAUNCH_I8S(float);
        else SN_LAUNCH_I8S(double);
#undef SN_LAUNCH_I8S
        if (int rc = check_launch("sn_conv_bank(i8s)")) return rc;
    }
    if (s.route && s.tol > 0.0f) {
        sn::GateScope guard(s.route, 1);
        return sn::conv_bank_group(x, SN_U8, bank, lambdas, B, Z, X, Y, G, Gtot, g0, head, kz, kx, ky, act, out,
                                   out_dtype, reinterpret_cast<sn_stream_t>(stream));
    }
    return SN_OK;
}

int conv_occ_i8z(const uint8_t* x, const float* bank, const float* lambdas, uint8_t* prep, int B, int Z, int X, int Y,
                 int G, int Gtot, int g0, int head, int kz, int kx, int ky, void* act, void* out, int out_dtype,
                 hipStream_t stream, int assume_served) {
    if (ky != 9 || kz != 9 || kx != 9 || Y % 16 != 0 || (reinterpret_cast<uintptr_t>(x) & 15) != 0 || G > 16) return 1;
    if ((long long)Z * X * Y >= (1ll << 31)) return 1;
    if (act && (reinterpret_cast<uintptr_t>(act) & 15)) return 1;
    if (out && (reinterpret_cast<uintptr_t>(out) & 15)) return 1;
    if (!prep || (reinterpret_cast<uintptr_t>(prep) & 15)) return 1;
    if (sn::option(sn::kOptConvSkipEmptyTiles) || !sn::option(sn::kOptConvI8Fold) || sn::option(sn::kOptConvI8Legacy)) return 1;
    const int cus = num_cus();
    Shape s4;
    memset(&s4, 0, sizeof(s4));
    s4.B = B; s4.Z = Z; s4.X = X; s4.Y = Y; s4.G = G; s4.kz = kz; s4.kx = kx;
    s4.Gtot = Gtot; s4.g0 = g0; s4.head = head;
    s4.gate = sn::current_gate();
    s4.nyt = (Y + TY - 1) / TY;
    s4.dynamic = 1;
    if (!plan_stride4(s4, B, Z, X, Y, kz, kx, cus)) return 1;
    s4.tol = sn::conv_i8_tolerance();
    s4.route = nullptr;
    int32_t* const route = reinterpret_cast<int32_t*>(prep + kPrepRoute);
    fp32k::ConvShape cs;
    bool dbl = false;
    if (!fp32k::plan_fp32(cs, B, Z, X, Y, G, Gtot, g0, head, kz, kx, ky, cus, false, dbl)) return 1;
    ZShape z;
    memset(&z, 0, sizeof(z));
    z.B = B; z.Z = Z; z.X = X; z.Y = Y; z.G = G; z.Gtot = Gtot; z.g0 = g0; z.head = head;
    z.gate = s4.gate;
    z.tol = s4.tol;
    z.route = route;
    z.dbg = sn::option(sn::kOptConvI8zInjectFault) ? 1 : 0;
    z.dense = sn::option(sn::kOptConvI8zDense) ? 1 : 0;
    z.served = assume_served ? 1 : 0;
    z.sticky = sn::sticky_device_ptr(stream);
    s4.sticky = z.sticky;
    z.nxt = (X + kZTX - 1) / kZTX;
    z.nyt = (Y + TY - 1) / TY;
    const long long ncol = (long long)B * z.nxt * z.nyt;
    if (ncol > (long long)cus * kZMaxJobs) return 1;
    int best_seg = 1;
    long long best_cost = -1;
    const int max_seg = (Z + 7) / 8;
    for (int ns = 1; ns <= max_seg; ++ns) {
        const int lz = (Z + ns - 1) / ns;
        const int nseg = (Z + lz - 1) / lz;
        const long long jobs = ncol * nseg;
        const long long per_wg = (jobs + cus - 1) / cus;
        if (per_wg > kZMaxJobs) continue;
        const long long cost = per_wg * (lz + 8) + kZD;
        if (best_cost < 0 || cost < best_cost) { best_cost = cost; best_seg = ns; }
    }
    if (best_cost < 0) return 1;
    if (!z.dense && SN_I8Z_SKIP_NSEG > 0 && SN_I8Z_SKIP_NSEG <= max_seg &&
        (ncol * SN_I8Z_SKIP_NSEG + cus - 1) / cus <= kZMaxJobs) {
        best_seg = SN_I8Z_SKIP_NSEG;
        z.deal = 1;
        z.deal_shift = SN_I8Z_SKIP_SHIFT;
    }
    z.LZ = (Z + best_seg - 1) / best_seg;
    z.nseg = (Z + z.LZ - 1) / z.LZ;
    z.PL = z.LZ + 8;
    const long long njobs = ncol * z.nseg;
    if (njobs > 0x7fffffff) return 1;
    z.njobs = (int)njobs;
    const int grid = (int)(njobs < cus ? njobs : cus);
    const int per_wg = (z.njobs + grid - 1) / grid;
    if (per_wg > kZMaxJobs) return 1;
    if (!division_magic((unsigned)z.PL, (unsigned)(per_wg * z.PL + 64), z.pl_magic)) return 1;
    z.swizzle = (grid % 8 == 0) ? 1 : 0;
    const size_t lds = lds_bytes_zwalk();
    const size_t lds_4 = lds_bytes(s4), lds_f = fp32k::lds_bytes(cs, false);
    const size_t lds_fb = lds_4 > lds_f ? lds_4 : lds_f;
    if (lds > (size_t)kMaxLds || lds_fb > (size_t)kMaxLds) return 1;
    hipEvent_t t_start = nullptr, t_stop = nullptr;
    sn::take_timing_events(t_start, t_stop);
#define SN_LAUNCH_I8Z(OT, KH, KR, KW)                                                                            \
    do {                                                                                                         \
        auto kern = act ? conv_occ_i8z_kernel<OT, KH, KR, KW, true> : conv_occ_i8z_kernel<OT, KH, KR, KW, false>; \
        if (sn::ensure_dynamic_lds((const void*)kern, kMaxLds) != hipSuccess)                                    \
            return check_launch("sn_conv_bank_prepared(i8z: hipFuncSetAttribute)");                              \
        if (t_start || t_stop)               \
            hipExtLaunchKernelGGL(kern, dim3(grid), dim3(64 * KW), (uint32_t)lds, stream, t_start, t_stop, 0u, x, lambdas,  \
                                  (const uint8_t*)prep, z, (OT*)act, (OT*)out);                                   \
        else                                                                                                     \
            hipLaunchKernelGGL(kern, dim3(grid), dim3(64 * KW), lds, stream, x, lambdas, (const uint8_t*)prep, z,   \
                               (OT*)act, (OT*)out);                                                              \
    } while (0)
#define SN_LAUNCH_I8Z_V(KH, KR, KW)                                                                              \
    do {                                                                                                         \
        if (out_dtype == SN_F32) SN_LAUNCH_I8Z(float, KH, KR, KW);                                               \
        else SN_LAUNCH_I8Z(double, KH, KR, KW);                                                                  \
    } while (0)
    switch (sn::option(sn::kOptConvI8zVariant)) {
        case 0: SN_LAUNCH_I8Z_V(2, 1, 8); break;
        case 1: SN_LAUNCH_I8Z_V(1, 1, 12); break;
        default: SN_LAUNCH_I8Z_V(1, 2, 12); break;
    }
#undef SN_LAUNCH_I8Z_V
#undef SN_LAUNCH_I8Z
    if (int rc = check_launch("sn_conv_bank_prepared(i8z)")) return rc;
    if (!assume_served) {
        const int fgrid = cus;
#define SN_LAUNCH_FB(OT)                                                                                         \
    do {                                                                                                         \
        auto kern = conv_i8_fallback_kernel<OT>;                                                                 \
        if (sn::ensure_dynamic_lds((const void*)kern, kMaxLds) != hipSuccess)                                    \
            return check_launch("sn_conv_bank_prepared(fallback: hipFuncSetAttribute)");                         \
        hipLaunchKernelGGL(kern, dim3(fgrid), dim3(kThreads), lds_fb, stream, x, bank, lambdas, (const int32_t*)route, s4, \
                           cs, (OT*)act, (OT*)out);                                                              \
    } while (0)
        if (out_dtype == SN_F32) SN_LAUNCH_FB(float);
        else SN_LAUNCH_FB(double);
#undef SN_LAUNCH_FB
    }
    return check_launch("sn_conv_bank_prepared(fallback)");
}

}

int sn::conv_occ_i8s_plan(int B, int Z, int X, int Y, int G, int kz, int kx, int ky, int32_t* plan8) {
    if (!stride4_shape(Y, G, kz, kx, ky)) return 1;
    Shape s;
    memset(&s, 0, sizeof(s));
    s.B = B; s.Z = Z; s.X = X; s.Y = Y; s.G = G; s.kz = kz; s.kx = kx;
    s.nyt = (Y + TY - 1) / TY;
    const int cus = num_cus();
    if (!plan_stride4(s, B, Z, X, Y, kz, kx, cus)) return 1;
    size_t ldsf = 0;
    plan8[0] = fold_fits(s, ldsf) ? 3 : 2;
    plan8[1] = s.TZ; plan8[2] = s.TX; plan8[3] = s.ntiles;
    plan8[4] = 2;
    plan8[5] = 4 * DW;
    plan8[6] = cus; plan8[7] = 0;
    return 0;
}

extern "C" int sn_conv_bank_prep(const float* bank, int G, int kz, int kx, int ky, void* prep, sn_stream_t stream) {
    if (!bank || !prep) return sn::fail(SN_ERR_INVALID_ARG, "sn_conv_bank_prep: null pointer");
    if (G <= 0 || kz <= 0 || kx <= 0 || ky <= 0) return sn::fail(SN_ERR_INVALID_ARG, "sn_conv_bank_prep: non-positive extent");
    if (reinterpret_cast<uintptr_t>(prep) & 15) return sn::fail(SN_ERR_INVALID_ARG, "sn_conv_bank_prep: prep must be 16-byte aligned");
    if (kz != 9 || kx != 9 || ky != 9) return SN_OK;
    for (int g0 = 0; g0 < G; g0 += 16) {
        const int gc = (G - g0 < 16) ? G - g0 : 16;
        hipLaunchKernelGGL(conv_prep_kernel, dim3(16), dim3(kPrepThreads), 0, sn::as_stream(stream), bank + (size_t)g0 * 729, gc,
                           static_cast<uint8_t*>(prep) + (size_t)(g0 / 16) * SN_CONV_PREP_BYTES);
    }
    return sn::check_launch("sn_conv_bank_prep");
}

static int conv_bank_prepared_impl(const void* x, int x_dtype, const float* bank, const float* lambdas, void* prep,
                                   int B, int Z, int X, int Y, int G, int kz, int kx, int ky, void* act, void* out,
                                   int out_dtype, sn_stream_t stream, int assume_served) {
    if (!x || !bank) return sn::fail(SN_ERR_INVALID_ARG, "sn_conv_bank_prepared: null x or bank");
    if (!act && !out) return sn::fail(SN_ERR_INVALID_ARG, "sn_conv_bank_prepared: both act and out are null");
    if (out && !lambdas) return sn::fail(SN_ERR_INVALID_ARG, "sn_conv_bank_prepared: out needs lambdas");
    if (B <= 0 || Z <= 0 || X <= 0 || Y <= 0 || G <= 0 || kz <= 0 || kx <= 0 || ky <= 0)
        return sn::fail(SN_ERR_INVALID_ARG, "sn_conv_bank_prepared: non-positive extent");
    if (out_dtype != SN_F32 && out_dtype != SN_F64)
        return sn::fail(SN_ERR_INVALID_ARG, "sn_conv_bank_prepared: out_dtype %d", out_dtype);
    if (x_dtype != SN_OCC8 || !prep || kz != 9 || kx != 9 || ky != 9 || (size_t)B * Z * X * Y > (size_t)1 << 40)
        return sn_conv_bank(x, x_dtype, bank, lambdas, B, Z, X, Y, G, kz, kx, ky, act, out, out_dtype, stream);
    for (int g0 = 0; g0 < G; g0 += 16) {
        const int gc = (G - g0 < 16) ? G - g0 : 16;
        const int head = G > 16 ? ((g0 > 0 ? 1 : 0) | (g0 + gc >= G ? 2 : 0)) : 2;
        int rc = sn::conv_occ_i8z((const uint8_t*)x, bank + (size_t)g0 * 729, lambdas ? lambdas + g0 : nullptr,
                                  static_cast<uint8_t*>(prep) + (size_t)(g0 / 16) * SN_CONV_PREP_BYTES, B, Z, X, Y, gc, G,
                                  g0, head, kz, kx, ky, act, out, out_dtype, sn::as_stream(stream), assume_served);
        if (rc == 1)
            rc = sn::conv_bank_group(x, x_dtype, bank + (size_t)g0 * 729, lambdas ? lambdas + g0 : nullptr, B, Z, X, Y, gc,
                                     G, g0, head, kz, kx, ky, act, out, out_dtype, stream);
        if (rc != SN_OK) return rc;
    }
    return SN_OK;
}

extern "C" int sn_conv_bank_prepared(const void* x, int x_dtype, const float* bank, const float* lambdas, void* prep,
                                     int B, int Z, int X, int Y, int G, int kz, int kx, int ky, void* act, void* out,
                                     int out_dtype, sn_stream_t stream) {
    return conv_bank_prepared_impl(x, x_dtype, bank, lambdas, prep, B, Z, X, Y, G, kz, kx, ky, act, out, out_dtype, stream, 0);
}

extern "C" int sn_conv_bank_prepared_served(const void* x, int x_dtype, const float* bank, const float* lambdas, void* prep,
                                            int B, int Z, int X, int Y, int G, int kz, int kx, int ky, void* act,
                                            void* out, int out_dtype, sn_stream_t stream) {
    return conv_bank_prepared_impl(x, x_dtype, bank, lambdas, prep, B, Z, X, Y, G, kz, kx, ky, act, out, out_dtype, stream, 1);
}

extern "C" int sn_conv_prep_verdict_offset(void) { return kPrepRoute; }

extern "C" int sn_conv_i8_path_counts(unsigned long long* counts3) {
    if (!counts3) return sn::fail(SN_ERR_INVALID_ARG, "sn_conv_i8_path_counts: null pointer");
    unsigned long long h[4] = {0, 0, 0, 0};
    if (hipDeviceSynchronize() != hipSuccess || hipMemcpyFromSymbol(h, HIP_SYMBOL(g_fold_counts), sizeof(h)) != hipSuccess)
        return sn::check_launch("sn_conv_i8_path_counts");
    counts3[0] = h[0]; counts3[1] = h[1]; counts3[2] = h[2];
    return SN_OK;
}

extern "C" int sn_conv_i8z_round_counts(unsigned long long* counts2) {
    if (!counts2) return sn::fail(SN_ERR_INVALID_ARG, "sn_conv_i8z_round_counts: null pointer");
    unsigned long long h[2] = {0, 0};
    if (hipDeviceSynchronize() != hipSuccess || hipMemcpyFromSymbol(h, HIP_SYMBOL(g_zwalk_rounds), sizeof(h)) != hipSuccess)
        return sn::check_launch("sn_conv_i8z_round_counts");
    counts2[0] = h[0]; counts2[1] = h[1];
    return SN_OK;
}

extern "C" int sn_conv_i8_spin_timeouts(unsigned long long* count) {
    if (!count) return sn::fail(SN_ERR_INVALID_ARG, "sn_conv_i8_spin_timeouts: null pointer");
    unsigned long long h[4] = {0, 0, 0, 0};
    if (hipDeviceSynchronize() != hipSuccess || hipMemcpyFromSymbol(h, HIP_SYMBOL(g_fold_counts), sizeof(h)) != hipSuccess)
        return sn::check_launch("sn_conv_i8_spin_timeouts");
    *count = h[3];
    return SN_OK;
}

#ifdef SN_CONV_TIMING
extern "C" void sn_debug_i8s_times(unsigned long long* host) {
    (void)hipDeviceSynchronize();
    (void)hipMemcpyFromSymbol(host, HIP_SYMBOL(g_i8s_t), sizeof(unsigned long long) * 1024 * 16);
    (void)hipMemcpyFromSymbol(host + 1024 * 16, HIP_SYMBOL(g_i8s_w), sizeof(unsigned long long) * 1024 * 64);
}
#endif
```

### scene-net_amd/csrc/conv_i8z.inc

```

constexpr int kZTX = 8;
constexpr int kZRows = kZTX + 8;
constexpr int kZRing = 16;
#ifndef SN_I8Z_LAG
#define SN_I8Z_LAG 3
#endif
constexpr int kZLag = SN_I8Z_LAG;
constexpr int kZD = 8 + kZLag;
#ifndef SN_I8Z_DD
#define SN_I8Z_DD 4
#endif
constexpr int kZDD = SN_I8Z_DD;
constexpr int kZPre = kZD + kZDD;
constexpr int kZRawPlane = kZRows * DW * 4;
constexpr int kZYqRow = 256, kZYqPlane = kZRows * kZYqRow;
constexpr int kZYcRow = 64, kZYcPlane = kZRows * kZYcRow + 32;
constexpr int kZMaxJobs = 256;
#ifndef SN_I8Z_SKIP_NSEG
#define SN_I8Z_SKIP_NSEG 0
#endif
#ifndef SN_I8Z_SKIP_SHIFT
#define SN_I8Z_SKIP_SHIFT 0
#endif
#ifndef SN_I8Z_AHEAD
#define SN_I8Z_AHEAD 2
#endif
static_assert(kZRing == 16 && (kZYcPlane / 4) % 16 == 8, "ring and bank arithmetic below");
static_assert(kZRing - 8 - kZLag >= 2, "the readers of a plane ride at least two slots before its overwrite");
static_assert(kZPre <= kZRing, "the prologue's planes fit the raw ring");


struct ZJob {
    int b, x0, y0, zs;
};

struct ZShape {
    int B, Z, X, Y, G, Gtot, g0, head;
    int nxt, nyt, nseg, LZ, PL;
    int njobs;
    unsigned pl_magic;
    int swizzle;
    float tol;
    sn::Gate gate;
    int32_t* route;
    int served;
    int32_t* sticky;
    int dbg;
    int dense;
    int deal, deal_shift;
};

__device__ unsigned long long g_zwalk_rounds[2] = {0ull, 0ull};

__device__ __forceinline__ int zjob_id(const ZShape& z, int wg, int k, int grid) {
    const int base = k * grid;
    if (z.swizzle && base + grid <= z.njobs) return base + (wg & 7) * (grid >> 3) + (wg >> 3);
    return base + wg;
}

constexpr int kPrepThreads = SN_BANK_THREADS;
__global__ __launch_bounds__(kPrepThreads) void conv_prep_kernel(const float* __restrict__ bank, int G,
                                                                 uint8_t* __restrict__ prep) {
    __shared__ __align__(16) float w[732 + kPrepScratchWords];
    const int g = blockIdx.x, tid = threadIdx.x;
    const bool valid = g < G;
    for (int i = tid; i < 729; i += kPrepThreads) w[i] = valid ? bank[(size_t)g * 729 + i] : 0.0f;
    prep_one_kernel(w, w + 732, valid, g, prep, tid, kPrepThreads);
}

template <typename OT, typename SH>
__device__ __forceinline__ void finish_round1(const SH& s, const TileCoord& c, int lx, int n, int q, int col, int q16,
                                              i32x4 (&acc)[3][4], const float* scale, const float* lamsc, const float* lamhi,
                                              OT* __restrict__ act, OT* __restrict__ out, size_t V) {
    const int gz = c.z0;
    const int gx = c.x0 + lx;
    if (gz >= s.Z || gx >= s.X) return;
    const int gy4 = c.y0 + 4 * n;
    float pm[4];
    const float4 lam4 = *reinterpret_cast<const float4*>(reinterpret_cast<const uint8_t*>(lamsc) + q16);
    const float lam[4] = {lam4.x, lam4.y, lam4.z, lam4.w};
    if (act) {
        float val[4][4];
#pragma unroll
        for (int v = 0; v < 4; ++v)
#pragma unroll
            for (int r = 0; r < 4; ++r) {
                const int low = acc[1][v][r] * 256 + acc[0][v][r];
                val[v][r] = fmaf((float)acc[2][v][r], 65536.0f, (float)low);
            }
        const float4 sc4 = *reinterpret_cast<const float4*>(scale + 4 * q);
        const float sc[4] = {sc4.x, sc4.y, sc4.z, sc4.w};
        if (gy4 < s.Y) {
#pragma unroll
            for (int r = 0; r < 4; ++r) {
                const int g = 4 * q + r;
                if (g < s.G) {
                    OT* o = act + ((size_t)c.b * s.Gtot + s.g0 + g) * V + ((size_t)gz * s.X + gx) * s.Y + gy4;
                    const float v0 = val[0][r] * sc[r], v1 = val[1][r] * sc[r], v2 = val[2][r] * sc[r], v3 = val[3][r] * sc[r];
                    if constexpr (sizeof(OT) == 4) {
                        *reinterpret_cast<float4*>(o) = make_float4(v0, v1, v2, v3);
                    } else {
                        reinterpret_cast<double2*>(o)[0] = make_double2((double)v0, (double)v1);
                        reinterpret_cast<double2*>(o)[1] = make_double2((double)v2, (double)v3);
                    }
                }
            }
        }
    }
    {
        using f32x2 = __attribute__((ext_vector_type(2))) float;
        const float4 hi4 = *reinterpret_cast<const float4*>(reinterpret_cast<const uint8_t*>(lamhi) + q16);
        const float lhi[4] = {hi4.x, hi4.y, hi4.z, hi4.w};
#pragma unroll
        for (int vp = 0; vp < 2; ++vp) {
            const int v0 = 2 * vp, v1 = 2 * vp + 1;
            f32x2 p = {0.0f, 0.0f};
#pragma unroll
            for (int r = 0; r < 4; ++r) {
                const int low0 = acc[1][v0][r] * 256 + acc[0][v0][r], low1 = acc[1][v1][r] * 256 + acc[0][v1][r];
                const f32x2 lo = {(float)low0, (float)low1};
                const f32x2 hi = {(float)acc[2][v0][r], (float)acc[2][v1][r]};
                p = __builtin_elementwise_fma(f32x2{lam[r], lam[r]}, lo, p);
                p = __builtin_elementwise_fma(f32x2{lhi[r], lhi[r]}, hi, p);
            }
            pm[v0] = p.x;
            pm[v1] = p.y;
        }
    }
    if (out) {
        auto sum_halves = [&](float a, float b) -> float {
            const auto r = __builtin_amdgcn_permlane32_swap(__float_as_uint(a), __float_as_uint(b), false, false);
            return __uint_as_float(r[0]) + __uint_as_float(r[1]);
        };
        auto sum_rows = [&](float u, float w) -> float {
            const auto r = __builtin_amdgcn_permlane16_swap(__float_as_uint(u), __float_as_uint(w), false, false);
            return __uint_as_float(r[0]) + __uint_as_float(r[1]);
        };
        const float e = sum_rows(sum_halves(pm[0], pm[2]), sum_halves(pm[1], pm[3]));
        const int gy = c.y0 + col;
        if (gy < s.Y) {
            OT* row = out + ((size_t)c.b * V + ((size_t)gz * s.X + gx) * s.Y + c.y0);
            OT* o = row + (unsigned)col;
            float t0 = e;
            if (s.head & 1) t0 += (float)load_now(o);
            if (s.head & 2) t0 = relu_tanh(t0);
            *o = (OT)t0;
        }
    }
}

template <typename OT>
__device__ __forceinline__ void zero_act_row(OT* o) {
    if constexpr (sizeof(OT) == 4) {
        *reinterpret_cast<float4*>(o) = make_float4(0.0f, 0.0f, 0.0f, 0.0f);
    } else {
        reinterpret_cast<double2*>(o)[0] = make_double2(0.0, 0.0);
        reinterpret_cast<double2*>(o)[1] = make_double2(0.0, 0.0);
    }
}
template <typename OT, typename SH>
__device__ __forceinline__ void zero_round1(const SH& s, const TileCoord& c, int lx, int n, int q, int col,
                                            OT* __restrict__ act, OT* __restrict__ out, size_t V) {
    const int gz = c.z0;
    const int gx = c.x0 + lx;
    if (gz >= s.Z || gx >= s.X) return;
    const int gy4 = c.y0 + 4 * n;
    if (act && gy4 < s.Y) {
#pragma unroll
        for (int r = 0; r < 4; ++r) {
            const int g = 4 * q + r;
            if (g < s.G) zero_act_row(act + ((size_t)c.b * s.Gtot + s.g0 + g) * V + ((size_t)gz * s.X + gx) * s.Y + gy4);
        }
    }
    if (out) {
        const int gy = c.y0 + col;
        if (gy < s.Y) {
            OT* row = out + ((size_t)c.b * V + ((size_t)gz * s.X + gx) * s.Y + c.y0);
            OT* o = row + (unsigned)col;
            float t0 = 0.0f;
            asm volatile("" : "+v"(t0));
            if (s.head & 1) t0 += (float)load_now(o);
            if (s.head & 2) t0 = relu_tanh(t0);
            *o = (OT)t0;
        }
    }
}
template <typename OT, typename SH>
__device__ __forceinline__ void zero_round2(const SH& s, const TileCoord& c, int lx, int n, int q, OT* __restrict__ act,
                                            OT* __restrict__ out, size_t V) {
    const int gz = c.z0;
    if (gz >= s.Z) return;
    const int gy4 = c.y0 + 4 * n;
    if (act && gy4 < s.Y) {
#pragma unroll
        for (int h = 0; h < 2; ++h) {
            const int gx = c.x0 + lx + h;
            if (gx < s.X) {
#pragma unroll
                for (int r = 0; r < 4; ++r) {
                    const int g = 4 * q + r;
                    if (g < s.G) zero_act_row(act + ((size_t)c.b * s.Gtot + s.g0 + g) * V + ((size_t)gz * s.X + gx) * s.Y + gy4);
                }
            }
        }
    }
    if (out) {
        const int h = q >> 1;
        const int gx = c.x0 + lx + h, gy = gy4 + 2 * (q & 1);
        if (gx < s.X && gy < s.Y) {
            OT* row = out + ((size_t)c.b * V + ((size_t)gz * s.X + (c.x0 + lx)) * s.Y + c.y0);
            OT* o = row + (unsigned)(h * s.Y + 4 * n + 2 * (q & 1));
            float t0 = 0.0f, t1 = 0.0f;
            asm volatile("" : "+v"(t0), "+v"(t1));
            if (s.head & 1) { t0 += (float)load_now(o); t1 += (float)load_now(o + 1); }
            if (s.head & 2) { t0 = relu_tanh(t0); t1 = relu_tanh(t1); }
            if constexpr (sizeof(OT) == 4) *reinterpret_cast<float2*>(o) = make_float2(t0, t1);
            else *reinterpret_cast<double2*>(o) = make_double2((double)t0, (double)t1);
        }
    }
}

constexpr uint32_t zrow_bits(uint32_t w) {
    return (w & 0xfu) | ((w & 0xf0u) << 4) | ((w & 0xf00u) << 8) | ((w & 0xf000u) << 12);
}
template <int kRows>
__device__ __forceinline__ uint32_t zwindow_mask(int c, int a) {
    constexpr uint32_t W = (1u << (8 + kRows)) - 1u;
    static_assert(kRows == 1 || kRows == 2, "a window of 9 or 10 rows: W << 3 stays inside 16 bits");
    const uint32_t m = c == 0 ? zrow_bits(W) : c == 1 ? zrow_bits(W << 1) : c == 2 ? zrow_bits(W << 2) : zrow_bits(W << 3);
    return m << (8 * a);
}

template <int kTag>
__device__ __forceinline__ void lds_add_lane0(int* counter, int value, int lane) {
    if (lane == 0) {
        const uint32_t a = (uint32_t)(uintptr_t)(__attribute__((address_space(3))) int*)counter;
        asm volatile("; @zw:add%c2\n\tds_add_u32 %0, %1" ::"v"(a), "v"(value), "i"(kTag) : "memory");
    }
}

template <typename OT, int kH, int kR, int kW, bool kAct>
__global__ __launch_bounds__(64 * kW) void conv_occ_i8z_kernel(const uint8_t* __restrict__ x,
                                                                const float* __restrict__ lambdas,
                                                                const uint8_t* __restrict__ prep, ZShape zs,
                                                                OT* __restrict__ act_arg, OT* __restrict__ out) {
    if (!zs.gate.pass()) return;
    OT* const act = kAct ? act_arg : nullptr;
    constexpr bool kLean = !kAct;
    extern __shared__ __attribute__((aligned(16))) uint8_t lds[];
    constexpr int kNT = 64 * kW;
    constexpr int kTPS = kZTX / (kH * kR);
    constexpr int kTShift = kTPS == 8 ? 3 : 2;
    constexpr int kNVz = 4 * kH;
    static_assert(kH == 1 || kH == 2, "rounds of one or two x-rows");
    static_assert(kTPS * kH * kR == kZTX && (kTPS == 8 || kTPS == 4), "ticket shape");
    const int tid = threadIdx.x;
    const int lane = tid & 63, wave = __builtin_amdgcn_readfirstlane(tid >> 6);
    uint4* Wd = reinterpret_cast<uint4*>(lds);
    int4* jobtab = reinterpret_cast<int4*>(Wd + kFoldSteps * 3 * 64);
    float* scale = reinterpret_cast<float*>(jobtab + kZMaxJobs);
    float* lamsc = scale + 16;
    float* lamhi = lamsc + 16;
    double* bnd = reinterpret_cast<double*>(lamhi + 32);
    int* cnt = reinterpret_cast<int*>(bnd + 16);
    int4* chk = reinterpret_cast<int4*>(cnt + 128);
    int4* ltab = chk + 64;
    int4* stab = ltab + 64;
    uint32_t* rowmask = reinterpret_cast<uint32_t*>(stab + 64);
    uint8_t* raw = reinterpret_cast<uint8_t*>(rowmask + 32);
    uint8_t* Yc = raw + kZRing * kZRawPlane;
    uint8_t* Yq = Yc + kZRing * kZYcPlane;
    int* const ticket_ctr = cnt + 96;

#ifdef SN_CONV_TIMING
    if (lane < 8 && wave < 8) g_i8s_w[(blockIdx.x * 8 + wave) * 8 + lane] = 0;
#define SN_ZT(k, t0) do { if (lane == 0 && wave < 8) g_i8s_w[(blockIdx.x * 8 + wave) * 8 + (k)] += clock64() - (t0); } while (0)
#define SN_ZNOW() clock64()
#else
#define SN_ZT(k, t0) do { (void)(t0); } while (0)
#define SN_ZNOW() 0ull
#endif
    SN_ST(0);
    const size_t V = (size_t)zs.Z * zs.X * zs.Y;
    const int grid = (int)gridDim.x;
    const int my_jobs = (int)blockIdx.x < zs.njobs ? (zs.njobs - 1 - (int)blockIdx.x) / grid + 1 : 0;
    const int NPL = my_jobs * zs.PL;
    const int nslots = NPL + kZD;
    if (tid < 128) cnt[tid] = 0;
    if (tid >= 128 && tid < 192) {
        const int l = tid - 128, i = l & 15, role = l >> 4;
        int4 e = make_int4(0, 0, 0, 0);
        if (role == 0 && i <= 8) e = make_int4(i - kZD, 0, 1, 2);
        if (role == 1 && i <= 8) e = make_int4(i - kZRing + kZLag, 16, 2, kTShift);
        if (l == 32) e = make_int4(0, 32, 2 | 0x30, 0);
        if (l == 40) e = make_int4(kZDD - 16, 0, 4, 2);
        if (l == 48) e = make_int4(-kZRing, 16, 8, kTShift);
        chk[l] = e;
    }
    if (tid >= 192 && tid < 256) {
        const int l = tid - 192;
        ltab[l] = make_int4((l & 15) * 16, (l >> 4) * 256, 4 * (l & 15) + (l >> 4), (l >> 4) * 16);
    }
    if (tid >= 256 && tid < 320) {
        const int e = tid - 256, sg = e >> 2, qq = e & 3;
        const int a = (sg + 2 * qq) & 15, b = (sg + 2 * qq + 1) & 15;
        const int yq0 = (int)(uint32_t)(uintptr_t)(__attribute__((address_space(3))) uint8_t*)Yq;
        const int yc0 = (int)(uint32_t)(uintptr_t)(__attribute__((address_space(3))) uint8_t*)Yc;
        stab[e] = make_int4(yq0 + a * kZYqPlane, yc0 + a * kZYcPlane, yq0 + b * kZYqPlane, yc0 + b * kZYcPlane);
    }
    if (tid < my_jobs) {
        int j = zjob_id(zs, (int)blockIdx.x, tid, grid);
        int xt, yt, sg;
        if (zs.deal) {
            const int ncol = zs.B * zs.nxt * zs.nyt;
            sg = j / ncol; j -= sg * ncol;
            xt = j % zs.nxt; j /= zs.nxt;
            yt = j % zs.nyt; j /= zs.nyt;
            xt = (xt + zs.deal_shift * sg) % zs.nxt;
        } else {
            xt = j % zs.nxt; j /= zs.nxt;
            yt = j % zs.nyt; j /= zs.nyt;
            sg = j % zs.nseg; j /= zs.nseg;
        }
        jobtab[tid] = make_int4(j, xt * kZTX, yt * TY, sg * zs.LZ);
    }
    lds_barrier();

    struct JobRegs { int k, b, x0, y0, zs; };
    auto job_fetch = [&](JobRegs& jr, int k) -> bool {
        if (k == jr.k) return false;
        const int4 jb = jobtab[k];
        jr.b = __builtin_amdgcn_readfirstlane(jb.x); jr.x0 = __builtin_amdgcn_readfirstlane(jb.y);
        jr.y0 = __builtin_amdgcn_readfirstlane(jb.z); jr.zs = __builtin_amdgcn_readfirstlane(jb.w);
        jr.k = k;
        return true;
    };
    JobRegs jd{-1, 0, 0, 0, 0}, jr{-1, 0, 0, 0, 0};
    const uint8_t* xb = x;
    OT* ob = nullptr;

    auto dma_pass = [&](int u, int xr, int ln) {
        const int dl_row = (ln * 43) >> 8, dl_i = ln - dl_row * kRowPieces;
        const int k = (int)__umulhi((unsigned)u, zs.pl_magic), p = u - k * zs.PL;
        const bool new_job = job_fetch(jd, k);
        if constexpr (kLean) {
            if (new_job) xb = x + (size_t)jd.b * V;
        }
        const int gz = jd.zs - 4 + p;
        const int gx = jd.x0 - 4 + 4 * xr + dl_row, gy = jd.y0 - PYA + 16 * dl_i;
        const bool ok = (unsigned)gz < (unsigned)zs.Z && (unsigned)gx < (unsigned)zs.X && (unsigned)gy < (unsigned)zs.Y;
        uint8_t* const dst = raw + (u & 15) * kZRawPlane + xr * (4 * DW * 4);
        const uint32_t lds_uni = __builtin_amdgcn_readfirstlane((uint32_t)(uintptr_t)(__attribute__((address_space(3))) uint8_t*)dst);
        const uint8_t* const tile = kLean ? xb : x + (size_t)jd.b * V;
        const uint8_t* src = ok ? tile + (unsigned)((gz * zs.X + gx) * zs.Y + gy) : prep + kPrepZero;
        if (ln < 4 * kRowPieces) {
            uint32_t m0_saved;
            asm volatile("; @zw:dma\n\ts_mov_b32 %0, m0\n\ts_mov_b32 m0, %1\n\ts_nop 0\n\tglobal_load_lds_dwordx4 %2, off\n\t"
                         "s_mov_b32 m0, %0"
                         : "=&s"(m0_saved) : "s"(lds_uni), "v"(src) : "memory");
        }
    };
    auto fold_pass = [&](int u, int xr, int ln) {
        const int n = ln & 15, q = ln >> 4;
        const uint32_t* p = reinterpret_cast<const uint32_t*>(raw + (u & 15) * kZRawPlane + (4 * xr + q) * (DW * 4) + (n + D0) * 4);
        const uint32_t R0 = p[0], R1 = p[1], R2 = p[2];
        const unsigned long long any = __builtin_amdgcn_ballot_w64((R0 | R1 | R2) != 0u);
        unsigned long long any4;
        uint32_t rowbits;
        asm("s_quadmask_b64 %0, %1" : "=s"(any4) : "s"(any) : "scc");
        asm("s_quadmask_b32 %0, %1" : "=s"(rowbits) : "s"((uint32_t)any4) : "scc");
        uint4 f;
        f.x = R0 + __builtin_amdgcn_perm(R2, R1, 0x01020304u);
        f.y = __builtin_amdgcn_alignbyte(R1, R0, 1) + __builtin_amdgcn_perm(R2, R1, 0x02030405u);
        f.z = __builtin_amdgcn_alignbyte(R1, R0, 2) + __builtin_amdgcn_perm(R2, R1, 0x03040506u);
        f.w = __builtin_amdgcn_alignbyte(R1, R0, 3) + __builtin_amdgcn_perm(R2, R1, 0x04050607u);
        *reinterpret_cast<uint4*>(Yq + (u & 15) * kZYqPlane + (4 * xr + q) * kZYqRow + n * 16) = f;
        *reinterpret_cast<uint32_t*>(Yc + (u & 15) * kZYcPlane + (4 * xr + q) * kZYcRow + n * 4) = R1;
        if (lane == 0) reinterpret_cast<uint8_t*>(rowmask)[(u & 15) * 4 + xr] = (uint8_t)rowbits;
    };

    auto poison_jobs = [&]() {
        const OT nan = (OT)__int_as_float(0x7fc00000);
        for (int k = 0; k < my_jobs; ++k) {
            const int4 jb = jobtab[k];
            for (int r = wave; r < zs.LZ * kZTX; r += kW) {
                const int gz = jb.w + (r >> 3), gx = jb.y + (r & 7), gy = jb.z + lane;
                if (gz >= zs.Z || gx >= zs.X || gy >= zs.Y) continue;
                const size_t off = ((size_t)gz * zs.X + gx) * zs.Y + gy;
                if (out) out[(size_t)jb.x * V + off] = nan;
                if (act)
                    for (int g = 0; g < zs.G; ++g) act[((size_t)jb.x * zs.Gtot + zs.g0 + g) * V + off] = nan;
            }
        }
    };

    const int npre = NPL < kZPre ? NPL : kZPre;
    for (int p = wave; p < 4 * npre; p += kW) dma_pass(p >> 2, p & 3, lane);
    {
        const uint4* src = reinterpret_cast<const uint4*>(prep + kPrepWd);
        for (int i = tid; i < kFoldSteps * 3 * 64; i += kNT) Wd[i] = src[i];
        if (tid < 16) {
            scale[tid] = reinterpret_cast<const float*>(prep + kPrepScale)[tid];
            bnd[tid] = reinterpret_cast<const double*>(prep + kPrepBnd)[tid];
            lamhi[16 + tid] = (lambdas && tid < zs.G) ? lambdas[tid] : 0.0f;
            if (tid < zs.G && reinterpret_cast<const int*>(prep + kPrepSym)[tid] == 0) cnt[97] = 1;
        }
        if (tid >= 64 && tid < 128) cnt[32 + tid - 64] = (((tid - 64) & 15) < npre && !((zs.dbg & 1) && tid == 64)) ? 1 : 0;
    }
    lds_barrier();
    {
        const bool asym = cnt[97] != 0;
        const bool exceeded = !asym && bound_exceeded<OT>(zs, bnd, lamhi + 16, act, out);
        if (blockIdx.x == 0 && tid == 0) {
            if (zs.route) *zs.route = asym ? 2 : exceeded ? 1 : 0;
            atomicAdd(&g_fold_counts[asym ? 1 : exceeded ? 2 : 0], 1ull);
        }
        if (asym || exceeded) {
            asm volatile("s_waitcnt vmcnt(0)" ::: "memory");
            if (zs.served) {
                poison_jobs();
                if (tid == 0) sn::sticky_latch(zs.sticky, 2, (int)blockIdx.x, asym ? 2 : 1);
            }
            return;
        }
    }
    if (wave == 0) {
        bool fin = true;
        if (tid < 16) {
            const float sc = scale[tid];
            const float ls = (out && tid < zs.G) ? lamhi[16 + tid] * sc : 0.0f;
            const float lh = 65536.0f * ls;
            lamsc[tid] = ls;
            lamhi[tid] = lh;
            auto finite = [](float v) { return (__float_as_uint(v) & 0x7f800000u) != 0x7f800000u; };
            fin = finite(sc) && !(__float_as_uint(sc) >> 31) && finite(ls) && finite(lh);
        }
        const bool all_fin = __builtin_amdgcn_ballot_w64(!fin) == 0ull;
        if (lane == 0) cnt[99] = (all_fin && !zs.dense) ? 1 : 0;
    }
    asm volatile("s_waitcnt vmcnt(0)" ::: "memory");
    __syncthreads();
    if (my_jobs == 0) return;
    const bool can_skip = __builtin_amdgcn_readfirstlane(cnt[99]) != 0;
    int n_run = 0, n_skip = 0;
    SN_ST(4);

    bool healthy = true;
    const int ntickets = kTPS * nslots;
    auto claim = [&]() -> int {
        int t = 0;
        if (lane == 0) t = __hip_atomic_fetch_add(ticket_ctr, 1, __ATOMIC_RELAXED, __HIP_MEMORY_SCOPE_WORKGROUP);
        return __builtin_amdgcn_readfirstlane(t);
    };
    int pend = -1;
    auto signal_passes = [&](int first) { lds_add_lane0<1>(&cnt[first], 1, lane); };

    int next = claim();
    for (int t = next; t < ntickets; t = next) {
        const unsigned long long tz0 = SN_ZNOW();
        next = claim();
        int ln = lane;
        asm volatile("" : "+v"(ln));
        const int s = t >> kTShift, tk = t & (kTPS - 1);
        int4 LT, ST;
        if constexpr (!kLean) {
            LT = ltab[ln];
            ST = *reinterpret_cast<const int4*>(reinterpret_cast<const uint8_t*>(stab) + ((s - kZD) & 15) * 64 + (ln & 0x30));
        }
        const bool pass_ticket = kTPS <= 4 || (tk & 1) == 0;
        const int xr0 = kTPS == 8 ? tk >> 1 : tk;
        const int sd = s + kZDD;
        const bool has_dma = pass_ticket && s >= kZD && sd < NPL;
        const bool has_fold = pass_ticket && s < NPL;
        const int sigma = s - kZD;
        int kr = 0, o = 0;
        bool has_round = false;
        if (sigma >= 0) {
            kr = (int)__umulhi((unsigned)sigma, zs.pl_magic);
            o = sigma - kr * zs.PL;
            has_round = o < zs.LZ;
        }
        if (pend >= 0) {
            asm volatile("; @zw:wait1\n\ts_waitcnt vmcnt(0)" ::: "memory");
            signal_passes(pend);
            pend = -1;
        }
        SN_ZT(0, tz0);
        const unsigned long long tz1 = SN_ZNOW();
        int midx;
        {
            const int4 role = chk[ln];
            const int have = (has_round ? 1 : 0) | (has_fold ? 2 : 0) | (has_dma ? 4 : 0) | 8;
            const int v = s + role.x;
            const int idx = ((v & 15) | role.y) + (role.z & (xr0 * 16));
            const int expect = ((role.z & have) && v >= 0) ? (((v >> 4) + 1) << role.w) : 0;
            midx = idx;
            int spins = 0;
            while (true) {
                const int seen = reinterpret_cast<const volatile __attribute__((address_space(3))) int*>(
                    (__attribute__((address_space(3))) int*)cnt)[idx];
                if (__builtin_amdgcn_ballot_w64(seen < expect) == 0ull) break;
                if (++spins > kSpinMax ||
                    ((spins & 63) == 0 &&
                     reinterpret_cast<const volatile __attribute__((address_space(3))) int*>((__attribute__((address_space(3))) int*)cnt)[98] != 0)) {
                    healthy = false;
                    break;
                }
                __builtin_amdgcn_s_sleep(2);
            }
            asm volatile("; @zw:spin_exit" ::: "memory");
        }
        if (!healthy) {
            if (lane == 0) {
                reinterpret_cast<volatile __attribute__((address_space(3))) int*>((__attribute__((address_space(3))) int*)cnt)[98] = 1;
                sn::sticky_latch(zs.sticky, 1, (int)blockIdx.x, t);
            }
            break;
        }
        SN_ZT(1, tz1);
        const unsigned long long tz2 = SN_ZNOW();
        const uint32_t rmask = reinterpret_cast<const volatile __attribute__((address_space(3))) uint32_t*>(
            (__attribute__((address_space(3))) uint32_t*)rowmask)[midx];
        if (has_dma) {
            dma_pass(sd, xr0, ln);
            pend = 32 + xr0 * 16 + (sd & 15);
        }
        if (has_fold) {
            fold_pass(s, xr0, ln);
            lds_add_lane0<2>(&cnt[s & 15], 1, lane);
        }
        SN_ZT(2, tz2);
        if (!has_round) {
            asm volatile("; @zw:wait3\n\ts_waitcnt lgkmcnt(0)" ::: "memory");
            lds_add_lane0<3>(&cnt[16 + (s & 15)], 1, lane);
            continue;
        }
        const unsigned long long tz3 = SN_ZNOW();
        const bool new_job = job_fetch(jr, kr);
        if constexpr (kLean) {
            if (new_job && out) ob = out + (size_t)jr.b * V;
        }
        const int gz = jr.zs + o;
        const int lx = kH * kR * tk;
        int rows_left = 0, nvalid = 0;
        if (gz >= zs.Z || jr.x0 + lx >= zs.X) {
            asm volatile("; @zw:wait3\n\ts_waitcnt lgkmcnt(0)" ::: "memory");
            lds_add_lane0<3>(&cnt[16 + (s & 15)], 1, lane);
            continue;
        }
        if constexpr (kLean) {
            rows_left = zs.X - (jr.x0 + lx);
            nvalid = rows_left >= kH * kR ? kR : (rows_left + kH - 1) / kH;
        }
        if (kLean && can_skip) {
            const uint32_t ub = zwindow_mask<kH * kR>(kH * kR == 2 ? (tk & 1) * 2 : (tk & 3), kH * kR == 2 ? tk >> 1 : tk >> 2);
            if (((uint32_t)__builtin_amdgcn_ballot_w64((rmask & ub) != 0u) & 0x1ffu) == 0u) {
                asm volatile("; @zw:wait3\n\ts_waitcnt lgkmcnt(0)" ::: "memory");
                lds_add_lane0<3>(&cnt[16 + (s & 15)], 1, lane);
                n_skip += nvalid;
                if (ob && (zs.head & 1)) {
                    TileCoord c;
                    c.b = 0; c.x0 = jr.x0; c.y0 = jr.y0; c.z0 = gz;
                    const int n = ln & 15, q = ln >> 4;
#pragma unroll 1
                    for (int rr = 0; rr < nvalid; ++rr) {
                        if constexpr (kH == 2) zero_round2<OT>(zs, c, lx + rr * kH, n, q, act, ob, V);
                        else zero_round1<OT>(zs, c, lx + rr * kH, n, q, 4 * n + q, act, ob, V);
                    }
                }
                if (ob && !(zs.head & 1)) {
                    OT* const row = ob + (unsigned)((gz * zs.X + jr.x0 + lx) * zs.Y);
                    float z0 = 0.0f;
                    asm volatile("" : "+v"(z0));
                    const OT zero = (OT)z0;
                    if (kH * kR == 2 && rows_left >= 2 && zs.nyt == 1) {
                        if (ln < zs.Y) {
                            OT* const o2 = row + 2u * (unsigned)ln;
                            if constexpr (sizeof(OT) == 4) *reinterpret_cast<float2*>(o2) = make_float2(zero, zero);
                            else *reinterpret_cast<double2*>(o2) = make_double2(zero, zero);
                        }
                    } else {
                        const int gy = jr.y0 + ln;
                        if (gy < zs.Y) {
                            row[(unsigned)gy] = zero;
                            if (kH * kR == 2 && rows_left >= 2) row[(unsigned)(zs.Y + gy)] = zero;
                        }
                    }
                }
                SN_ZT(6, tz0);
                continue;
            }
        }
        TileCoord c;
        c.b = kLean ? 0 : jr.b; c.x0 = jr.x0; c.y0 = jr.y0; c.z0 = gz;
        OT* const oq = kLean ? ob : out;
        if constexpr (kLean) {
            LT = ltab[ln];
            ST = *reinterpret_cast<const int4*>(reinterpret_cast<const uint8_t*>(stab) + ((s - kZD) & 15) * 64 + (ln & 0x30));
        }
        const int lr = ln;
        const int n16 = LT.x, q256 = LT.y;
        __builtin_assume((n16 & 15) == 0 && (q256 & 255) == 0);
        const int n4 = n16 >> 2, q64 = q256 >> 2;
        const int n = n16 >> 4, q = q256 >> 8;
        using lds_cp = const __attribute__((address_space(3))) uint8_t*;
        auto at = [&](int a) { return (const uint8_t*)(lds_cp)(uintptr_t)(uint32_t)a; };
        const int s8 = (sigma + 8) & 15;
        const int uq = __builtin_amdgcn_readfirstlane(lx * kZYqRow), uc = __builtin_amdgcn_readfirstlane(lx * kZYcRow);
        const int u8q = __builtin_amdgcn_readfirstlane((int)(uint32_t)(uintptr_t)(lds_cp)Yq + s8 * kZYqPlane + lx * kZYqRow);
        const int u8c = __builtin_amdgcn_readfirstlane((int)(uint32_t)(uintptr_t)(lds_cp)Yc + s8 * kZYcPlane + lx * kZYcRow);
        const uint8_t* yqA = at(ST.x + n16 + uq);
        const uint8_t* yqB = at(ST.z + n16 + uq);
        const uint8_t* yq8 = at(u8q + n16);
        const uint8_t* ycA = at(ST.y + n4 + uc);
        const uint8_t* ycB = at(ST.w + n4 + uc);
        const uint8_t* yc8 = at(u8c + n4);

        auto load_unit = [&](auto SLOT, auto HC, uint32_t (&r)[10]) {
            constexpr int slot = decltype(SLOT)::value, h = decltype(HC)::value;
            constexpr bool single = fold_slot_single(slot / kFoldRows, slot % kFoldRows);
            const uint8_t *q1, *q2, *c1, *c2;
            if constexpr (slot == 8) {
                q1 = yq8 + (h + 4) * kZYqRow; c1 = yc8 + (h + 4) * kZYcRow;
                q2 = q1; c2 = c1;
            } else if constexpr (slot == 11) {
                q1 = yq8 + h * kZYqRow + q256; c1 = yc8 + h * kZYcRow + q64;
                q2 = yq8 + (h + 8) * kZYqRow - q256; c2 = yc8 + (h + 8) * kZYcRow - q64;
            } else {
                constexpr int dx = fold_slot_dx(slot);
                const uint8_t* bq = fold_slot_a(slot) ? yqB : yqA;
                const uint8_t* bc = fold_slot_a(slot) ? ycB : ycA;
                q1 = bq + (h + dx) * kZYqRow; c1 = bc + (h + dx) * kZYcRow;
                q2 = bq + (h + 8 - dx) * kZYqRow; c2 = bc + (h + 8 - dx) * kZYcRow;
            }
            const uint4 a = *reinterpret_cast<const uint4*>(q1);
            r[0] = a.x; r[1] = a.y; r[2] = a.z; r[3] = a.w;
            r[4] = *reinterpret_cast<const uint32_t*>(c1);
            if constexpr (!single) {
                const uint4 b = *reinterpret_cast<const uint4*>(q2);
                r[5] = b.x; r[6] = b.y; r[7] = b.z; r[8] = b.w;
                r[9] = *reinterpret_cast<const uint32_t*>(c2);
            }
        };
        auto fold_unit = [&](const uint32_t (&r)[10], auto SLOT, i32x4 (&X)[4], uint32_t& centre) {
            constexpr int slot = decltype(SLOT)::value, J = slot % kFoldRows;
            constexpr bool single = fold_slot_single(slot / kFoldRows, J);
            if constexpr (single) {
                X[0][J] = (int)r[0]; X[1][J] = (int)r[1]; X[2][J] = (int)r[2]; X[3][J] = (int)r[3];
                centre = r[4];
            } else {
                X[0][J] = (int)(r[0] + r[5]); X[1][J] = (int)(r[1] + r[6]);
                X[2][J] = (int)(r[2] + r[7]); X[3][J] = (int)(r[3] + r[8]);
                centre = r[4] + r[9];
            }
        };
        auto centres = [&](uint32_t c0, uint32_t c1, uint32_t c2, i32x4 (&X)[4]) {
            uint32_t ov[4];
            transpose3(c0, c1, c2, ov);
#pragma unroll
            for (int r = 0; r < 4; ++r) X[r][3] = (int)ov[r];
        };
        if constexpr (!kLean) {
            rows_left = zs.X - (c.x0 + lx);
            nvalid = rows_left >= kH * kR ? kR : (rows_left + kH - 1) / kH;
        }
        uint32_t hits[kR];
#pragma unroll
        for (int rr = 0; rr < kR; ++rr) {
            if (kLean && kR == 1) { hits[rr] = 1u; continue; }
            uint32_t wb;
            if constexpr (kLean) {
                wb = zwindow_mask<kH>((tk & 1) * 2 + rr, tk >> 1);
            } else {
                const uint32_t w = ((1u << (8 + kH)) - 1u) << (lx + rr * kH);
                wb = (w & 0xfu) | ((w & 0xf0u) << 4) | ((w & 0xf00u) << 8) | ((w & 0xf000u) << 12);
            }
            asm("" : "+s"(wb));
            hits[rr] = can_skip ? ((uint32_t)__builtin_amdgcn_ballot_w64((rmask & wb) != 0u) & 0x1ffu) : 1u;
        }
#pragma unroll 1
        for (int rr = 0; rr < nvalid; ++rr) {
            if ((kR == 1 || rr == 0 ? hits[0] : hits[kR - 1]) == 0u) {
                if (rr == nvalid - 1) {
                    asm volatile("; @zw:wait3\n\ts_waitcnt lgkmcnt(0)" ::: "memory");
                    lds_add_lane0<3>(&cnt[16 + (s & 15)], 1, lane);
                }
                if constexpr (kH == 2) zero_round2<OT>(zs, c, lx + rr * kH, n, q, act, oq, V);
                else zero_round1<OT>(zs, c, lx + rr * kH, n, q, LT.z, act, oq, V);
                ++n_skip;
                yqA += kH * kZYqRow; yqB += kH * kZYqRow; yq8 += kH * kZYqRow;
                ycA += kH * kZYcRow; ycB += kH * kZYcRow; yc8 += kH * kZYcRow;
                continue;
            }
            ++n_run;
            constexpr int ro = 0;
            constexpr int kNU = 3 * kH, kNP = 4 * kH;
            uint32_t praw[kNU][10], pcen[3][kH];
            auto pipe_load = [&](auto ST, auto UC) {
                constexpr int st = decltype(ST)::value, u = decltype(UC)::value;
                load_unit(std::integral_constant<int, st * kFoldRows + u / kH>{}, std::integral_constant<int, u % kH + ro>{}, praw[u]);
            };
            constexpr int kAhead = SN_I8Z_AHEAD;
            auto pipe_piece = [&](auto ST, auto PC, i32x4 (&X)[kH][4], auto NST) {
                constexpr int st = decltype(ST)::value, piece = decltype(PC)::value, nst = decltype(NST)::value;
                if constexpr (piece < kNU) {
                    constexpr int j = piece / kH, h = piece % kH;
                    fold_unit(praw[piece], std::integral_constant<int, st * kFoldRows + j>{}, X[h], pcen[j][h]);
                } else {
                    constexpr int h = piece - kNU;
                    centres(pcen[0][h], pcen[1][h], pcen[2][h], X[h]);
                }
                if constexpr (piece + kAhead < kNU) pipe_load(ST, std::integral_constant<int, piece + kAhead>{});
                else if constexpr (piece >= kNP - kAhead && nst >= 0 && piece - (kNP - kAhead) < kNU)
                    pipe_load(std::integral_constant<int, (nst < 0 ? 0 : nst)>{}, std::integral_constant<int, piece - (kNP - kAhead)>{});
            };
            constexpr std::integral_constant<int, 0> S0{};
            constexpr std::integral_constant<int, 1> S1{};
            constexpr std::integral_constant<int, 2> S2{};
            constexpr std::integral_constant<int, 3> S3{};
            constexpr std::integral_constant<int, -1> SNone{};

            i32x4 acc[3][kNVz];
            auto load_w = [&](int st, i32x4 (&w)[3]) {
#pragma unroll
                for (int d = 0; d < 3; ++d) {
                    const uint4 u = Wd[(st * 3 + d) * 64 + lr];
                    w[d] = i32x4{(int)u.x, (int)u.y, (int)u.z, (int)u.w};
                }
            };
            auto mma_tile = [&](const i32x4 (&w)[3], const i32x4& xv, int v, bool first) {
#pragma unroll
                for (int d = 0; d < 3; ++d)
                    acc[d][v] = __builtin_amdgcn_mfma_i32_16x16x64_i8(w[d], xv, first ? i32x4{0, 0, 0, 0} : acc[d][v], 0, 0, 0);
            };
            auto mma_step = [&](const i32x4 (&w)[3], const i32x4 (&X)[kH][4], bool first, auto&& work) {
                auto group = [&](auto VC) {
                    constexpr int v = decltype(VC)::value, h = v >> 2, r = v & 3;
                    mma_tile(w, X[h][r], v, first);
                    __builtin_amdgcn_sched_barrier(0);
                    work(VC);
                    __builtin_amdgcn_sched_barrier(0);
                };
                group(std::integral_constant<int, 0>{}); group(std::integral_constant<int, 1>{});
                group(std::integral_constant<int, 2>{}); group(std::integral_constant<int, 3>{});
                if constexpr (kH == 2) {
                    group(std::integral_constant<int, 4>{}); group(std::integral_constant<int, 5>{});
                    group(std::integral_constant<int, 6>{}); group(std::integral_constant<int, 7>{});
                }
            };
            i32x4 Xa[kH][4], Xb[kH][4];
            i32x4 wa[3], wb[3];
            load_w(0, wa);
            {
                auto all_units = [&](auto&& f) {
                    f(std::integral_constant<int, 0>{}); f(std::integral_constant<int, 1>{}); f(std::integral_constant<int, 2>{});
                    if constexpr (kH == 2) {
                        f(std::integral_constant<int, 3>{}); f(std::integral_constant<int, 4>{}); f(std::integral_constant<int, 5>{});
                    }
                };
                all_units([&](auto U) { pipe_load(S0, U); });
                all_units([&](auto U) {
                    constexpr int u = decltype(U)::value;
                    fold_unit(praw[u], std::integral_constant<int, u / kH>{}, Xa[u % kH], pcen[u / kH][u % kH]);
                });
#pragma unroll
                for (int h = 0; h < kH; ++h) centres(pcen[0][h], pcen[1][h], pcen[2][h], Xa[h]);
                auto first_ahead = [&](auto U) {
                    constexpr int u = decltype(U)::value;
                    if constexpr (u < kAhead && u < kNU) pipe_load(S1, U);
                };
                first_ahead(std::integral_constant<int, 0>{}); first_ahead(std::integral_constant<int, 1>{});
                first_ahead(std::integral_constant<int, 2>{}); first_ahead(std::integral_constant<int, 3>{});
            }
            load_w(1, wb);
            __builtin_amdgcn_sched_barrier(0);
            if (rr == 0) SN_ZT(3, tz3);
            const unsigned long long tz4 = SN_ZNOW();
            mma_step(wa, Xa, true, [&](auto v) { pipe_piece(S1, v, Xb, S2); });
            load_w(2, wa);
            __builtin_amdgcn_sched_barrier(0);
            mma_step(wb, Xb, false, [&](auto v) { pipe_piece(S2, v, Xa, S3); });
            load_w(3, wb);
            __builtin_amdgcn_sched_barrier(0);
            mma_step(wa, Xa, false, [&](auto v) { pipe_piece(S3, v, Xb, SNone); });
            __builtin_amdgcn_sched_barrier(0);
            if (rr == nvalid - 1) {
                asm volatile("; @zw:wait3\n\ts_waitcnt lgkmcnt(0)" ::: "memory");
                lds_add_lane0<3>(&cnt[16 + (s & 15)], 1, lane);
            }
            mma_step(wb, Xb, false, [](auto) {});
            if (pend >= 0) {
                asm volatile("; @zw:wait1\n\ts_waitcnt vmcnt(0)" ::: "memory");
                signal_passes(pend);
                pend = -1;
            }
            SN_ZT(4, tz4);
            const unsigned long long tz5 = SN_ZNOW();
            if constexpr (kH == 2 && kLean) {
                int le = lr;
                asm volatile("" : "+v"(le));
                finish_round<OT>(zs, c, 0, lx + rr * kH, le & 15, le >> 4, acc, scale, lamsc, lamhi, act, oq, V);
            } else if constexpr (kH == 2) finish_round<OT>(zs, c, 0, lx + rr * kH, n, q, acc, scale, lamsc, lamhi, act, oq, V);
            else finish_round1<OT>(zs, c, lx + rr * kH, n, q, LT.z, LT.w, acc, scale, lamsc, lamhi, act, oq, V);
            SN_ZT(5, tz5);
            yqA += kH * kZYqRow; yqB += kH * kZYqRow; yq8 += kH * kZYqRow;
            ycA += kH * kZYcRow; ycB += kH * kZYcRow; yc8 += kH * kZYcRow;
        }
        SN_ZT(6, tz0);
    }
    SN_ST(5);
    if (pend >= 0) {
        asm volatile("; @zw:wait1\n\ts_waitcnt vmcnt(0)" ::: "memory");
        signal_passes(pend);
    }
    if (lane == 0) {
        const uint32_t a = (uint32_t)(uintptr_t)(__attribute__((address_space(3))) int*)(cnt + 100);
        asm volatile("ds_add_u32 %0, %1\n\tds_add_u32 %0, %2 offset:4" ::"v"(a), "v"(n_run), "v"(n_skip) : "memory");
        if (atomicInc(reinterpret_cast<unsigned*>(cnt + 102), 0xffffffffu) == (unsigned)kW - 1u) {
            const volatile __attribute__((address_space(3))) int* tot = (__attribute__((address_space(3))) int*)cnt;
            atomicAdd(&g_zwalk_rounds[0], (unsigned long long)(unsigned)tot[100]);
            atomicAdd(&g_zwalk_rounds[1], (unsigned long long)(unsigned)tot[101]);
        }
    }
    asm volatile("s_waitcnt vmcnt(0)" ::: "memory");
    if (reinterpret_cast<const volatile __attribute__((address_space(3))) int*>((__attribute__((address_space(3))) int*)cnt)[98] != 0) {
        __syncthreads();
        poison_jobs();
        if (!healthy && lane == 0) atomicAdd(&g_fold_counts[3], 1ull);
    }
}

template <typename OT>
__global__ __launch_bounds__(kThreads) void conv_i8_fallback_kernel(const uint8_t* __restrict__ x,
                                                                    const float* __restrict__ bank,
                                                                    const float* __restrict__ lambdas,
                                                                    const int32_t* __restrict__ route, Shape s4,
                                                                    fp32k::ConvShape cs, OT* __restrict__ act,
                                                                    OT* __restrict__ out) {
    if (!cs.gate.pass()) return;
    const int verdict = *route;
    if (verdict <= 0) return;
    bool to_fp32 = verdict == 1;
    if (verdict == 2) {
        to_fp32 = conv_occ_i8s_body<OT, 10, 6, 1>(x, bank, lambdas, s4, act, out);
        if (to_fp32) __syncthreads();
    }
    if (to_fp32) fp32k::conv_bank_body<uint8_t, OT, false>(x, bank, lambdas, cs, act, out);
}

size_t lds_bytes_zwalk() {
    return (size_t)kFoldSteps * 3 * 64 * 16 + (size_t)kZMaxJobs * 16 + 64 * 4 + 128 + 128 * 4 + 64 * 16 + 2 * 64 * 16 +
           32 * 4 + (size_t)kZRing * (kZRawPlane + kZYcPlane + kZYqPlane) + 16;
}

bool division_magic(unsigned d, unsigned umax, unsigned& magic) {
    magic = (unsigned)((((unsigned long long)1 << 32) / d) + 1ull);
    for (unsigned u = 0; u <= umax; ++u)
        if ((unsigned)(((unsigned long long)u * magic) >> 32) != u / d) return false;
    return true;
}
```

Before: 275,700 tiles/s.

## Add census pre-pass to deal only live z-segment jobs and zero-fill dead ones

Adds a census kernel that scans the occupancy grid per batch and short z-segment, and records which x-tiles have any occupied voxels in their receptive window. The main i8 z-walk conv kernel reads this plan, re-deals only the live (segment, x-tile) jobs across workgroups using shorter segments, and writes zeros directly for dead tiles. This replaces the previous static skip-deal heuristic. The aim is to stop spending matrix-core rounds and DMA on empty regions of sparse point-cloud grids, at the cost of an extra launch, a workspace allocation per call, and more halo overhead from the shorter segments.

```diff
diff --git a/include/scenenet_hip.h b/include/scenenet_hip.h
--- a/include/scenenet_hip.h
+++ b/include/scenenet_hip.h
@@ -74,6 +74,12 @@
                                  int B, int Z, int X, int Y, int G, int kz, int kx, int ky,
                                  void* act, void* out, int out_dtype, sn_stream_t stream);
 int sn_conv_prep_verdict_offset(void);
+int sn_conv_bank_planned(const void* x, int x_dtype, const float* bank, const float* lambdas, void* prep,
+                         int B, int Z, int X, int Y, int G, int kz, int kx, int ky,
+                         void* act, void* out, int out_dtype, sn_stream_t stream, void* ws, size_t ws_bytes,
+                         int assume_served);
+size_t sn_conv_plan_ws_bytes(int B, int Z, int X, int Y);
+int sn_conv_i8z_plan_counts(unsigned long long* counts4);
 int sn_conv_i8_spin_timeouts(unsigned long long* count);
 int sn_conv_i8z_round_counts(unsigned long long* counts2);
 int sn_voxel_onepass_giveups(unsigned long long* count);
diff --git a/scene-net_amd/_hip.py b/scene-net_amd/_hip.py
--- a/scene-net_amd/_hip.py
+++ b/scene-net_amd/_hip.py
@@ -40,6 +40,10 @@
     "sn_conv_prep_verdict_offset": (c_int, []),
     "sn_conv_i8_spin_timeouts": (c_int, [_P]),
     "sn_conv_i8z_round_counts": (c_int, [_P]),
+    "sn_conv_bank_planned": (c_int, [_P, _I, _P, _P, _P, _I, _I, _I, _I, _I, _I, _I, _I, _P, _P, _I, _P, _P, ctypes.c_size_t,
+                                     _I]),
+    "sn_conv_plan_ws_bytes": (ctypes.c_size_t, [_I, _I, _I, _I]),
+    "sn_conv_i8z_plan_counts": (c_int, [_P]),
     "sn_voxel_onepass_giveups": (c_int, [_P]),
     "sn_launch_timing_events": (c_int, [_P, _P]),
     "sn_conv_fused": (c_int, [_P, _I, _P, _P, _I, _I, _I, _I, _I, _I, _I, _I, _P, _I, _P]),
@@ -248,6 +252,12 @@
     return int(buf[0])
 
 
+def conv_i8z_plan_counts() -> Tuple[int, int, int, int]:
+    buf = (ctypes.c_ulonglong * 4)()
+    _check(load().sn_conv_i8z_plan_counts(ctypes.cast(buf, ctypes.c_void_p)), "sn_conv_i8z_plan_counts")
+    return int(buf[0]), int(buf[1]), int(buf[2]), int(buf[3])
+
+
 def conv_i8z_round_counts() -> Tuple[int, int]:
     buf = (ctypes.c_ulonglong * 2)()
     _check(load().sn_conv_i8z_round_counts(ctypes.cast(buf, ctypes.c_void_p)), "sn_conv_i8z_round_counts")
@@ -458,12 +468,14 @@
     if prep is not None:
         if prep.dtype != torch.uint8 or prep.numel() < SN_CONV_PREP_BYTES * ((G + 15) // 16):
             raise HipLibraryError("prep: not a blob of conv_bank_prep for this bank")
-        fn = load().sn_conv_bank_prepared_served if assume_served else load().sn_conv_bank_prepared
-        rc = fn(_ptr(x, None, "x"), _DT[x.dtype], _ptr(bank, torch.float32, "bank"),
-                _ptr(lambdas, torch.float32, "lambdas"), _ptr(prep, torch.uint8, "prep"),
-                B, Z, X, Y, G, kz, kx, ky, _ptr(act, None, "act"), _ptr(out, None, "out"),
-                _DT_OUT[out_dtype], _stream())
-        _check(rc, "sn_conv_bank_prepared")
+        nws = load().sn_conv_plan_ws_bytes(B, Z, X, Y)
+        ws = torch.empty(nws, dtype=torch.uint8, device=x.device) if nws else None
+        rc = load().sn_conv_bank_planned(_ptr(x, None, "x"), _DT[x.dtype], _ptr(bank, torch.float32, "bank"),
+                                         _ptr(lambdas, torch.float32, "lambdas"), _ptr(prep, torch.uint8, "prep"),
+                                         B, Z, X, Y, G, kz, kx, ky, _ptr(act, None, "act"), _ptr(out, None, "out"),
+                                         _DT_OUT[out_dtype], _stream(), _ptr(ws, torch.uint8, "ws"), nws,
+                                         1 if assume_served else 0)
+        _check(rc, "sn_conv_bank_planned")
         return act, out
     rc = load().sn_conv_bank(_ptr(x, None, "x"), _DT[x.dtype], _ptr(bank, torch.float32, "bank"),
                              _ptr(lambdas, torch.float32, "lambdas"), B, Z, X, Y, G, kz, kx, ky,
diff --git a/scene-net_amd/csrc/cabi.hip b/scene-net_amd/csrc/cabi.hip
--- a/scene-net_amd/csrc/cabi.hip
+++ b/scene-net_amd/csrc/cabi.hip
@@ -36,6 +36,7 @@
     {"corr_dense",             "SN_CORR_DENSE",         1,  0,       0,  1,       true},
     {"corr_sparse_tile_bytes", nullptr,                 0,  0,       0,  2048,    false},
     {"conv_i8z_inject_fault",  nullptr,                 0,  0,       0,  1,       true},
+    {"conv_i8z_plan",          nullptr,                 0,  0,       0,  2,       false},
     {"conv_i8z_dense",         nullptr,                 0,  0,       0,  1,       true},
 };
 static_assert(sizeof(g_options) / sizeof(g_options[0]) == kOptCount, "one entry per sn::Opt");
diff --git a/scene-net_amd/csrc/common.h b/scene-net_amd/csrc/common.h
--- a/scene-net_amd/csrc/common.h
+++ b/scene-net_amd/csrc/common.h
@@ -42,6 +42,7 @@
     kOptCorrDense,
     kOptCorrSparseTileBytes,
     kOptConvI8zInjectFault,
+    kOptConvI8zPlan,
     kOptConvI8zDense,
     kOptCount
 };
diff --git a/scene-net_amd/csrc/conv_i8s.hip b/scene-net_amd/csrc/conv_i8s.hip
--- a/scene-net_amd/csrc/conv_i8s.hip
+++ b/scene-net_amd/csrc/conv_i8s.hip
@@ -1,5 +1,7 @@
 #include "common.h"
+#include "scan.h"
 #include <hip/hip_ext.h>
+#include <atomic>
 #include <cstdlib>
 #include <cstring>
 #include <type_traits>
@@ -129,6 +131,8 @@
 }
 
 #include "conv_i8z.inc"
+
+std::atomic<unsigned long long> g_plan_static_host{0};
 
 }
 
@@ -217,9 +221,16 @@
     return SN_OK;
 }
 
+size_t conv_plan_ws_bytes(int B, int Z, int X, int Y) {
+    if (B <= 0 || Z <= 0 || X <= 0 || Y <= 0 || X > 64 || Y > 64 || Y % 16 != 0) return 0;
+    const long long words = (long long)B * ((Z + 7) / 8);
+    if (words > kZPlanMaxWords) return 0;
+    return (size_t)(kZPlanHdr + 2 * words) * 4;
+}
+
 int conv_occ_i8z(const uint8_t* x, const float* bank, const float* lambdas, uint8_t* prep, int B, int Z, int X, int Y,
                  int G, int Gtot, int g0, int head, int kz, int kx, int ky, void* act, void* out, int out_dtype,
-                 hipStream_t stream, int assume_served) {
+                 hipStream_t stream, int assume_served, void* ws, size_t ws_bytes) {
     if (ky != 9 || kz != 9 || kx != 9 || Y % 16 != 0 || (reinterpret_cast<uintptr_t>(x) & 15) != 0 || G > 16) return 1;
     if ((long long)Z * X * Y >= (1ll << 31)) return 1;
     if (act && (reinterpret_cast<uintptr_t>(act) & 15)) return 1;
@@ -269,29 +280,51 @@
         if (best_cost < 0 || cost < best_cost) { best_cost = cost; best_seg = ns; }
     }
     if (best_cost < 0) return 1;
-    if (!z.dense && SN_I8Z_SKIP_NSEG > 0 && SN_I8Z_SKIP_NSEG <= max_seg &&
-        (ncol * SN_I8Z_SKIP_NSEG + cus - 1) / cus <= kZMaxJobs) {
-        best_seg = SN_I8Z_SKIP_NSEG;
-        z.deal = 1;
-        z.deal_shift = SN_I8Z_SKIP_SHIFT;
-    }
     z.LZ = (Z + best_seg - 1) / best_seg;
     z.nseg = (Z + z.LZ - 1) / z.LZ;
     z.PL = z.LZ + 8;
     const long long njobs = ncol * z.nseg;
     if (njobs > 0x7fffffff) return 1;
     z.njobs = (int)njobs;
-    const int grid = (int)(njobs < cus ? njobs : cus);
+    int grid = (int)(njobs < cus ? njobs : cus);
+    const int variant = sn::option(sn::kOptConvI8zVariant), plan_opt = sn::option(sn::kOptConvI8zPlan);
+    bool offered = ws && plan_opt != 0 && !z.dense && !act && out && !(head & 1) && variant == 2 && sn::conv_plan_ws_bytes(B, Z, X, Y) != 0 &&
+                   (reinterpret_cast<uintptr_t>(ws) & 15) == 0;
+    if (offered) {
+        z.LZd = SN_I8Z_PLAN_LZ < z.LZ ? SN_I8Z_PLAN_LZ : z.LZ;
+        z.nsegd = (Z + z.LZd - 1) / z.LZd;
+        z.PLd = z.LZd + 8;
+        const long long nwords = (long long)B * z.nsegd, njobs_d = nwords * z.nxt;
+        offered = nwords <= kZPlanMaxWords && ws_bytes >= (size_t)(kZPlanHdr + 2 * nwords) * 4;
+        if (offered) {
+            const int grid_d = (int)(njobs_d < cus ? njobs_d : cus);
+            const int g = grid > grid_d ? grid : grid_d;
+            const int per_wg_d = (int)((njobs_d + g - 1) / g);
+            offered = per_wg_d + 1 <= kZMaxJobs &&
+                      division_magic((unsigned)z.PLd, (unsigned)(per_wg_d * z.PLd + 64), z.pld_magic);
+            if (offered) grid = g;
+        }
+    }
     const int per_wg = (z.njobs + grid - 1) / grid;
     if (per_wg > kZMaxJobs) return 1;
     if (!division_magic((unsigned)z.PL, (unsigned)(per_wg * z.PL + 64), z.pl_magic)) return 1;
     z.swizzle = (grid % 8 == 0) ? 1 : 0;
+    z.st_planes = per_wg * z.PL;
+    z.plan_ws = offered ? static_cast<const uint32_t*>(ws) : nullptr;
+    z.plan_mode = plan_opt;
     const size_t lds = lds_bytes_zwalk();
     const size_t lds_4 = lds_bytes(s4), lds_f = fp32k::lds_bytes(cs, false);
     const size_t lds_fb = lds_4 > lds_f ? lds_4 : lds_f;
     if (lds > (size_t)kMaxLds || lds_fb > (size_t)kMaxLds) return 1;
     hipEvent_t t_start = nullptr, t_stop = nullptr;
     sn::take_timing_events(t_start, t_stop);
+    if (offered) {
+        hipLaunchKernelGGL(conv_census_kernel, dim3(2 * B * z.nsegd), dim3(kCensusThreads), 0, stream, x, lambdas,
+                           (const uint8_t*)prep, z, static_cast<uint32_t*>(ws));
+        if (int rc = check_launch("sn_conv_bank_planned(census)")) return rc;
+    } else {
+        g_plan_static_host.fetch_add(1, std::memory_order_relaxed);
+    }
 #define SN_LAUNCH_I8Z(OT, KH, KR, KW)                                                                            \
     do {                                                                                                         \
         auto kern = act ? conv_occ_i8z_kernel<OT, KH, KR, KW, true> : conv_occ_i8z_kernel<OT, KH, KR, KW, false>; \
@@ -309,7 +342,7 @@
         if (out_dtype == SN_F32) SN_LAUNCH_I8Z(float, KH, KR, KW);                                               \
         else SN_LAUNCH_I8Z(double, KH, KR, KW);                                                                  \
     } while (0)
-    switch (sn::option(sn::kOptConvI8zVariant)) {
+    switch (variant) {
         case 0: SN_LAUNCH_I8Z_V(2, 1, 8); break;
         case 1: SN_LAUNCH_I8Z_V(1, 1, 12); break;
         default: SN_LAUNCH_I8Z_V(1, 2, 12); break;
@@ -368,7 +401,8 @@
 
 static int conv_bank_prepared_impl(const void* x, int x_dtype, const float* bank, const float* lambdas, void* prep,
                                    int B, int Z, int X, int Y, int G, int kz, int kx, int ky, void* act, void* out,
-                                   int out_dtype, sn_stream_t stream, int assume_served) {
+                                   int out_dtype, sn_stream_t stream, int assume_served, void* ws = nullptr,
+                                   size_t ws_bytes = 0) {
     if (!x || !bank) return sn::fail(SN_ERR_INVALID_ARG, "sn_conv_bank_prepared: null x or bank");
     if (!act && !out) return sn::fail(SN_ERR_INVALID_ARG, "sn_conv_bank_prepared: both act and out are null");
     if (out && !lambdas) return sn::fail(SN_ERR_INVALID_ARG, "sn_conv_bank_prepared: out needs lambdas");
@@ -383,7 +417,8 @@
         const int head = G > 16 ? ((g0 > 0 ? 1 : 0) | (g0 + gc >= G ? 2 : 0)) : 2;
         int rc = sn::conv_occ_i8z((const uint8_t*)x, bank + (size_t)g0 * 729, lambdas ? lambdas + g0 : nullptr,
                                   static_cast<uint8_t*>(prep) + (size_t)(g0 / 16) * SN_CONV_PREP_BYTES, B, Z, X, Y, gc, G,
-                                  g0, head, kz, kx, ky, act, out, out_dtype, sn::as_stream(stream), assume_served);
+                                  g0, head, kz, kx, ky, act, out, out_dtype, sn::as_stream(stream), assume_served, ws,
+                                  ws_bytes);
         if (rc == 1)
             rc = sn::conv_bank_group(x, x_dtype, bank + (size_t)g0 * 729, lambdas ? lambdas + g0 : nullptr, B, Z, X, Y, gc,
                                      G, g0, head, kz, kx, ky, act, out, out_dtype, stream);
@@ -402,6 +437,24 @@
                                             int B, int Z, int X, int Y, int G, int kz, int kx, int ky, void* act,
                                             void* out, int out_dtype, sn_stream_t stream) {
     return conv_bank_prepared_impl(x, x_dtype, bank, lambdas, prep, B, Z, X, Y, G, kz, kx, ky, act, out, out_dtype, stream, 1);
+}
+
+extern "C" int sn_conv_bank_planned(const void* x, int x_dtype, const float* bank, const float* lambdas, void* prep, int B,
+                                    int Z, int X, int Y, int G, int kz, int kx, int ky, void* act, void* out, int out_dtype,
+                                    sn_stream_t stream, void* ws, size_t ws_bytes, int assume_served) {
+    return conv_bank_prepared_impl(x, x_dtype, bank, lambdas, prep, B, Z, X, Y, G, kz, kx, ky, act, out, out_dtype, stream,
+                                   assume_served ? 1 : 0, ws, ws_bytes);
+}
+
+extern "C" size_t sn_conv_plan_ws_bytes(int B, int Z, int X, int Y) { return sn::conv_plan_ws_bytes(B, Z, X, Y); }
+
+extern "C" int sn_conv_i8z_plan_counts(unsigned long long* counts4) {
+    if (!counts4) return sn::fail(SN_ERR_INVALID_ARG, "sn_conv_i8z_plan_counts: null pointer");
+    unsigned long long h[4] = {0, 0, 0, 0};
+    if (hipDeviceSynchronize() != hipSuccess || hipMemcpyFromSymbol(h, HIP_SYMBOL(g_zwalk_plan), sizeof(h)) != hipSuccess)
+        return sn::check_launch("sn_conv_i8z_plan_counts");
+    counts4[0] = h[0]; counts4[1] = h[1] + g_plan_static_host.load(std::memory_order_relaxed); counts4[2] = h[2]; counts4[3] = h[3];
+    return SN_OK;
 }
 
 extern "C" int sn_conv_prep_verdict_offset(void) { return kPrepRoute; }
diff --git a/scene-net_amd/csrc/conv_i8z.inc b/scene-net_amd/csrc/conv_i8z.inc
--- a/scene-net_amd/csrc/conv_i8z.inc
+++ b/scene-net_amd/csrc/conv_i8z.inc
@@ -16,12 +16,11 @@
 constexpr int kZYqRow = 256, kZYqPlane = kZRows * kZYqRow;
 constexpr int kZYcRow = 64, kZYcPlane = kZRows * kZYcRow + 32;
 constexpr int kZMaxJobs = 256;
-#ifndef SN_I8Z_SKIP_NSEG
-#define SN_I8Z_SKIP_NSEG 0
+#ifndef SN_I8Z_PLAN_LZ
+#define SN_I8Z_PLAN_LZ 16
 #endif
-#ifndef SN_I8Z_SKIP_SHIFT
-#define SN_I8Z_SKIP_SHIFT 0
-#endif
+constexpr int kZPlanHdr = 4;
+constexpr int kZPlanMaxWords = 768;
 #ifndef SN_I8Z_AHEAD
 #define SN_I8Z_AHEAD 2
 #endif
@@ -47,10 +46,15 @@
     int32_t* sticky;
     int dbg;
     int dense;
-    int deal, deal_shift;
+    const uint32_t* plan_ws;
+    int plan_mode;
+    int nsegd, LZd, PLd;
+    unsigned pld_magic;
+    int st_planes;
 };
 
 __device__ unsigned long long g_zwalk_rounds[2] = {0ull, 0ull};
+__device__ unsigned long long g_zwalk_plan[4] = {0ull, 0ull, 0ull, 0ull};
 
 __device__ __forceinline__ int zjob_id(const ZShape& z, int wg, int k, int grid) {
     const int base = k * grid;
@@ -66,6 +70,71 @@
     const bool valid = g < G;
     for (int i = tid; i < 729; i += kPrepThreads) w[i] = valid ? bank[(size_t)g * 729 + i] : 0.0f;
     prep_one_kernel(w, w + 732, valid, g, prep, tid, kPrepThreads);
+}
+
+constexpr int kCensusThreads = 1024;
+__global__ __launch_bounds__(kCensusThreads) void conv_census_kernel(const uint8_t* __restrict__ x,
+                                                                     const float* __restrict__ lambdas,
+                                                                     const uint8_t* __restrict__ prep, ZShape zs,
+                                                                     uint32_t* __restrict__ ws) {
+    if (!zs.gate.pass()) return;
+    __shared__ unsigned long long s_rows[kCensusThreads / 64];
+    const int tid = threadIdx.x;
+    const int seg = (int)blockIdx.x >> 1, half = (int)blockIdx.x & 1;
+    const int b = seg / zs.nsegd, sg = seg - b * zs.nsegd;
+    const int z0 = sg * zs.LZd;
+    const int zlo = z0 - 4 < 0 ? 0 : z0 - 4, zhi = z0 + zs.LZd + 4 > zs.Z ? zs.Z : z0 + zs.LZd + 4;
+    const int row16 = zs.Y >> 4;
+    const int ppl = zs.X * row16;
+    const int np = zhi - zlo;
+    const int j = tid & 255, pg = 4 * half + (tid >> 8);
+    uint32_t any = 0u;
+    if (j < ppl) {
+        const uint4* src = reinterpret_cast<const uint4*>(x + (size_t)b * zs.Z * zs.X * zs.Y + (size_t)zlo * zs.X * zs.Y) + j;
+        for (int p = pg; p < np; p += 32) {
+            uint4 v[4];
+#pragma unroll
+            for (int u = 0; u < 4; ++u) {
+                const int pp = p + 8 * u;
+                v[u] = pp < np ? src[(size_t)pp * ppl] : make_uint4(0u, 0u, 0u, 0u);
+            }
+#pragma unroll
+            for (int u = 0; u < 4; ++u) any |= v[u].x | v[u].y | v[u].z | v[u].w;
+        }
+    }
+    unsigned long long rows = any ? 1ull << (j / row16) : 0ull;
+    rows = sn::wave_reduce(rows, [](unsigned long long a, unsigned long long c) { return a | c; });
+    if ((tid & 63) == 0) s_rows[tid >> 6] = rows;
+    __syncthreads();
+    if (tid == 0) {
+        unsigned long long all = 0ull;
+        for (int w = 0; w < kCensusThreads / 64; ++w) all |= s_rows[w];
+        uint32_t live = 0u;
+        for (int xt = 0; xt < zs.nxt; ++xt) {
+            const int lo = xt * kZTX - 4 < 0 ? 0 : xt * kZTX - 4, hi = xt * kZTX + 12 > zs.X ? zs.X : xt * kZTX + 12;
+            const unsigned long long win = ((1ull << (hi - lo)) - 1ull) << lo;
+            if (all & win) live |= 1u << xt;
+        }
+        ws[kZPlanHdr + blockIdx.x] = live;
+    }
+    if (blockIdx.x == 0 && tid < 64) {
+        bool fin = true, asym = false;
+        if (tid < 16) {
+            const float sc = reinterpret_cast<const float*>(prep + kPrepScale)[tid];
+            const float ls = tid < zs.G ? lambdas[tid] * sc : 0.0f;
+            const float lh = 65536.0f * ls;
+            auto finite = [](float v) { return (__float_as_uint(v) & 0x7f800000u) != 0x7f800000u; };
+            fin = finite(sc) && !(__float_as_uint(sc) >> 31) && finite(ls) && finite(lh);
+            asym = tid < zs.G && reinterpret_cast<const int*>(prep + kPrepSym)[tid] == 0;
+        }
+        const bool bad = __builtin_amdgcn_ballot_w64(!fin || asym) != 0ull;
+        if (tid == 0) {
+            const float* one = lambdas;
+            const bool exceeded = bound_exceeded<float>(zs, reinterpret_cast<const double*>(prep + kPrepBnd), lambdas,
+                                                        (const float*)nullptr, one);
+            ws[0] = (!bad && !exceeded && !zs.dense) ? 1u : 0u;
+        }
+    }
 }
 
 template <typename OT, typename SH>
@@ -283,9 +352,12 @@
     SN_ST(0);
     const size_t V = (size_t)zs.Z * zs.X * zs.Y;
     const int grid = (int)gridDim.x;
-    const int my_jobs = (int)blockIdx.x < zs.njobs ? (zs.njobs - 1 - (int)blockIdx.x) / grid + 1 : 0;
-    const int NPL = my_jobs * zs.PL;
-    const int nslots = NPL + kZD;
+    constexpr bool kPlan = kLean && kH == 1 && kR == 2 && kW == 12;
+    int my_jobs = (int)blockIdx.x < zs.njobs ? (zs.njobs - 1 - (int)blockIdx.x) / grid + 1 : 0;
+    int PL = zs.PL;
+    unsigned pl_magic = zs.pl_magic;
+    int my_dead = 0;
+    bool dealt = false;
     if (tid < 128) cnt[tid] = 0;
     if (tid >= 128 && tid < 192) {
         const int l = tid - 128, i = l & 15, role = l >> 4;
@@ -308,22 +380,65 @@
         const int yc0 = (int)(uint32_t)(uintptr_t)(__attribute__((address_space(3))) uint8_t*)Yc;
         stab[e] = make_int4(yq0 + a * kZYqPlane, yc0 + a * kZYcPlane, yq0 + b * kZYqPlane, yc0 + b * kZYcPlane);
     }
-    if (tid < my_jobs) {
+    if constexpr (kPlan) {
+        if (zs.plan_ws && !(zs.head & 1)) {
+            const int nwords = zs.B * zs.nsegd;
+            const uint32_t hdr = zs.plan_ws[0];
+            uint32_t word = 0u;
+            if (tid < nwords) {
+                const uint2 pair = reinterpret_cast<const uint2*>(zs.plan_ws + kZPlanHdr)[tid];
+                word = pair.x | pair.y;
+            }
+            int pre[1] = {(int)__builtin_popcount(word)};
+            const int n_live = __builtin_amdgcn_readfirstlane(sn::block_exclusive<kNT, 1, int>(pre, reinterpret_cast<int*>(raw)));
+            const int n_all = nwords * zs.nxt, n_dead = n_all - n_live;
+            const int per_wg = (n_live + grid - 1) / grid;
+            dealt = __builtin_amdgcn_readfirstlane(hdr) != 0u && (zs.plan_mode == 2 || per_wg * zs.PLd < zs.st_planes);
+            if (blockIdx.x == 0 && tid == 0) {
+                atomicAdd(&g_zwalk_plan[dealt ? 0 : 1], 1ull);
+                atomicAdd(&g_zwalk_plan[2], (unsigned long long)n_live);
+                atomicAdd(&g_zwalk_plan[3], (unsigned long long)n_dead);
+            }
+            if (dealt) {
+                const int wg = (int)blockIdx.x;
+                PL = zs.PLd; pl_magic = zs.pld_magic;
+                my_jobs = wg < n_live ? (n_live - 1 - wg) / grid + 1 : 0;
+                my_dead = wg < n_dead ? (n_dead - 1 - wg) / grid + 1 : 0;
+                if (tid < nwords) {
+                    const int LZ = PL - 8, b = tid / zs.nsegd, z0 = (tid - b * zs.nsegd) * LZ;
+                    int lq = pre[0] / grid, lm = pre[0] - lq * grid;
+                    const int d0 = tid * zs.nxt - pre[0];
+                    int dq = d0 / grid, dm = d0 - dq * grid;
+                    int dead_rounds = 0;
+                    const int nz = zs.Z - z0 < LZ ? zs.Z - z0 : LZ;
+                    for (int xt = 0; xt < zs.nxt; ++xt) {
+                        const int4 e = make_int4(b, xt * kZTX, 0, z0);
+                        if ((word >> xt) & 1u) {
+                            if (lm == wg) jobtab[lq] = e;
+                            if (++lm == grid) { lm = 0; ++lq; }
+                        } else {
+                            if (dm == wg) {
+                                jobtab[kZMaxJobs - 1 - dq] = e;
+                                dead_rounds += nz * (zs.X - xt * kZTX < kZTX ? zs.X - xt * kZTX : kZTX);
+                            }
+                            if (++dm == grid) { dm = 0; ++dq; }
+                        }
+                    }
+                    if (dead_rounds) atomicAdd(&g_zwalk_rounds[1], (unsigned long long)dead_rounds);
+                }
+            }
+        }
+    }
+    if (!dealt && tid < my_jobs) {
         int j = zjob_id(zs, (int)blockIdx.x, tid, grid);
         int xt, yt, sg;
-        if (zs.deal) {
-            const int ncol = zs.B * zs.nxt * zs.nyt;
-            sg = j / ncol; j -= sg * ncol;
-            xt = j % zs.nxt; j /= zs.nxt;
-            yt = j % zs.nyt; j /= zs.nyt;
-            xt = (xt + zs.deal_shift * sg) % zs.nxt;
-        } else {
-            xt = j % zs.nxt; j /= zs.nxt;
-            yt = j % zs.nyt; j /= zs.nyt;
-            sg = j % zs.nseg; j /= zs.nseg;
-        }
+        xt = j % zs.nxt; j /= zs.nxt;
+        yt = j % zs.nyt; j /= zs.nyt;
+        sg = j % zs.nseg; j /= zs.nseg;
         jobtab[tid] = make_int4(j, xt * kZTX, yt * TY, sg * zs.LZ);
     }
+    const int NPL = my_jobs * PL;
+    const int nslots = NPL + kZD;
     lds_barrier();
 
     struct JobRegs { int k, b, x0, y0, zs; };
@@ -341,7 +456,7 @@
 
     auto dma_pass = [&](int u, int xr, int ln) {
         const int dl_row = (ln * 43) >> 8, dl_i = ln - dl_row * kRowPieces;
-        const int k = (int)__umulhi((unsigned)u, zs.pl_magic), p = u - k * zs.PL;
+        const int k = (int)__umulhi((unsigned)u, pl_magic), p = u - k * PL;
         const bool new_job = job_fetch(jd, k);
         if constexpr (kLean) {
             if (new_job) xb = x + (size_t)jd.b * V;
@@ -379,11 +494,11 @@
         if (lane == 0) reinterpret_cast<uint8_t*>(rowmask)[(u & 15) * 4 + xr] = (uint8_t)rowbits;
     };
 
-    auto poison_jobs = [&]() {
+    auto poison_jobs = [&](int nj, int lz) {
         const OT nan = (OT)__int_as_float(0x7fc00000);
-        for (int k = 0; k < my_jobs; ++k) {
+        for (int k = 0; k < nj; ++k) {
             const int4 jb = jobtab[k];
-            for (int r = wave; r < zs.LZ * kZTX; r += kW) {
+            for (int r = wave; r < lz * kZTX; r += kW) {
                 const int gz = jb.w + (r >> 3), gx = jb.y + (r & 7), gy = jb.z + lane;
                 if (gz >= zs.Z || gx >= zs.X || gy >= zs.Y) continue;
                 const size_t off = ((size_t)gz * zs.X + gx) * zs.Y + gy;
@@ -417,8 +532,23 @@
         }
         if (asym || exceeded) {
             asm volatile("s_waitcnt vmcnt(0)" ::: "memory");
+            if constexpr (kPlan) {
+                if (dealt && zs.served) {
+                    __syncthreads();
+                    PL = zs.PL;
+                    my_jobs = (int)blockIdx.x < zs.njobs ? (zs.njobs - 1 - (int)blockIdx.x) / grid + 1 : 0;
+                    if (tid < my_jobs) {
+                        int j = zjob_id(zs, (int)blockIdx.x, tid, grid);
+                        const int xt = j % zs.nxt; j /= zs.nxt;
+                        const int yt = j % zs.nyt; j /= zs.nyt;
+                        const int sg = j % zs.nseg; j /= zs.nseg;
+                        jobtab[tid] = make_int4(j, xt * kZTX, yt * TY, sg * zs.LZ);
+                    }
+                    __syncthreads();
+                }
+            }
             if (zs.served) {
-                poison_jobs();
+                poison_jobs(my_jobs, PL - 8);
                 if (tid == 0) sn::sticky_latch(zs.sticky, 2, (int)blockIdx.x, asym ? 2 : 1);
             }
             return;
@@ -440,6 +570,25 @@
     }
     asm volatile("s_waitcnt vmcnt(0)" ::: "memory");
     __syncthreads();
+    auto zero_fill_dead = [&]() {
+        for (int k = 0; k < my_dead; ++k) {
+            const int4 jb = jobtab[kZMaxJobs - 1 - k];
+            const int nz = zs.Z - jb.w < PL - 8 ? zs.Z - jb.w : PL - 8, nr = zs.X - jb.y < kZTX ? zs.X - jb.y : kZTX;
+            const int per = nr * zs.Y >> 2;
+            OT* const base = out + (size_t)jb.x * V + (size_t)(jb.w * zs.X + jb.y) * zs.Y;
+            for (int i = tid; i < nz * per; i += kNT) {
+                const int zi = i / per, ci = i - zi * per;
+                OT* const o4 = base + (size_t)zi * zs.X * zs.Y + 4 * ci;
+                if constexpr (sizeof(OT) == 4) {
+                    *reinterpret_cast<float4*>(o4) = make_float4(0.0f, 0.0f, 0.0f, 0.0f);
+                } else {
+                    reinterpret_cast<double2*>(o4)[0] = make_double2(0.0, 0.0);
+                    reinterpret_cast<double2*>(o4)[1] = make_double2(0.0, 0.0);
+                }
+            }
+        }
+    };
+    if constexpr (kPlan) zero_fill_dead();
     if (my_jobs == 0) return;
     const bool can_skip = __builtin_amdgcn_readfirstlane(cnt[99]) != 0;
     int n_run = 0, n_skip = 0;
@@ -476,9 +625,9 @@
         int kr = 0, o = 0;
         bool has_round = false;
         if (sigma >= 0) {
-            kr = (int)__umulhi((unsigned)sigma, zs.pl_magic);
-            o = sigma - kr * zs.PL;
-            has_round = o < zs.LZ;
+            kr = (int)__umulhi((unsigned)sigma, pl_magic);
+            o = sigma - kr * PL;
+            has_round = o < PL - 8;
         }
         if (pend >= 0) {
             asm volatile("; @zw:wait1\n\ts_waitcnt vmcnt(0)" ::: "memory");
@@ -825,7 +974,7 @@
     asm volatile("s_waitcnt vmcnt(0)" ::: "memory");
     if (reinterpret_cast<const volatile __attribute__((address_space(3))) int*>((__attribute__((address_space(3))) int*)cnt)[98] != 0) {
         __syncthreads();
-        poison_jobs();
+        poison_jobs(kPlan ? (int)__umulhi((unsigned)NPL, pl_magic) : my_jobs, PL - 8);
         if (!healthy && lane == 0) atomicAdd(&g_fold_counts[3], 1ull);
     }
 }
```

Result: no change. 275,100 tiles/s, median of 2 (-0.2%).
